# RapidAI/RapidDoc

Measured on AMD Instinct MI355X. Metric: pages/sec (layout+OCR det/rec), higher is better.
Workload: dtype f32

## Files before the change

### include/rapiddoc_mi355.h

```cpp
#ifndef RAPIDDOC_MI355_H
#define RAPIDDOC_MI355_H

#include <stddef.h>
#include <stdint.h>

#ifdef __cplusplus
extern "C" {
#endif

typedef struct rd_handle rd_handle;

#define RD_REC_UNFUSED_CTC 1
#define RD_REC_WANT_SOFTMAX 2
#define RD_REC_WANT_LOGITS 4
#define RD_REC_WANT_NECK 64

const char* rd_version(void);
rd_handle* rd_create(int device_id, const char* model_kind);
const char* rd_create_error(void);
void rd_destroy(rd_handle* h);
const char* rd_last_error(rd_handle* h);

int rd_load_weights(rd_handle* h, const void* safetensors_image, size_t nbytes);

int rd_query_workspace(rd_handle* h, int B, int H, int W, int flags, size_t* ws_bytes);

int rd_det_forward(rd_handle* h, const float* x_nchw_dev, int B, int H, int W, float* prob_b1hw_dev, void* ws_dev,
                   size_t ws_bytes, void* stream);
#define RD_DET_WANT_NECK 1
int rd_det_forward_ex(rd_handle* h, const float* x_nchw_dev, int B, int H, int W, float* prob_b1hw_dev, int flags, float* aux_dev,
                      void* ws_dev, size_t ws_bytes, void* stream);

int rd_rec_forward(rd_handle* h, const float* x_nchw_dev, int B, int W, int32_t* idx_bt_dev, float* prob_bt_dev,
                   float* full_btc_dev, int flags, void* ws_dev, size_t ws_bytes, void* stream);
int rd_rec_num_classes(rd_handle* h);
#define RD_REC_STAGE_BACKBONE 8
#define RD_REC_STAGE_TAIL 16
int rd_rec_token_dim(rd_handle* h);
int rd_rec_backbone_forward(rd_handle* h, const float* x_nchw_dev, int B, int W, float* tokens_btd_dev, void* ws_dev, size_t ws_bytes,
                            void* stream);
int rd_rec_tail_forward(rd_handle* h, const float* tokens_dev, int n_tokens, int n_lines, int max_tokens, const int32_t* seg_dev,
                        const int32_t* tokinfo_dev, int32_t* idx_dev, float* prob_dev, void* ws_dev, size_t ws_bytes, void* stream);
#define RD_REC_LINE_WIDTHS 32
int rd_rec_backbone_forward_lines(rd_handle* h, const float* x_nchw_dev, int B, int W, const int32_t* line_tab_dev, float* tokens_dev,
                                  void* ws_dev, size_t ws_bytes, void* stream);
int rd_rec_seq_len(int W);

int rd_backbone_forward(rd_handle* h, const float* x_nchw_dev, int B, int H, int W, float* const feats_dev[4],
                        void* ws_dev, size_t ws_bytes, void* stream);

int rd_formula_encoder_forward(rd_handle* h, const float* x_nchw_dev, int B, int C, int H, int W, float* enc_dev,
                               void* ws_dev, size_t ws_bytes, void* stream);

int rd_formula_decode(rd_handle* h, const float* enc_dev, int B, int S, int max_new_tokens, int64_t* ids_dev, int32_t* n_cols,
                      void* stream);
#define RD_FORMULA_STREAM_MAX_SLOTS 32
#define RD_FORMULA_STREAM_MAX_TOKENS 65536
typedef struct rd_formula_stream_stats {
    int32_t steps;
    int32_t live_slot_steps;
    int32_t slots;
    int32_t admitted;
} rd_formula_stream_stats;
int rd_formula_decode_stream(rd_handle* h, const float* enc_dev, int N, int S, int max_new_tokens, int slots, int64_t* ids_dev,
                             int32_t* lens_dev, rd_formula_stream_stats* stats, void* stream);
int rd_formula_max_new_tokens(rd_handle* h);

int rd_preproc_resize_norm(int device_id, const uint8_t* hwc_u8_dev, int H, int W, int OH, int OW, const float mean[3],
                           const float std[3], float scale, int interp, int swap_rb, float* out_chw_dev, void* stream);

int rd_preproc_resize_norm_batch(int device_id, const uint8_t* pages_u8_dev, int P, int H, int W, int OH, int OW, const float mean[3],
                                 const float std[3], float scale, int interp, int swap_rb, float* out_nchw_dev, void* stream);

#define RD_RESIZE_AA_MAX_SIDE 16384
int rd_preproc_resize_aa_norm(int device_id, const uint8_t* hwc_u8_dev, int H, int W, int OH, int OW, const float mean[3],
                              const float std[3], int swap_rb, float* out_chw_dev, uint8_t* out_u8_hwc_dev, void* stream);

#define RD_RESAMPLE_BILINEAR 2
#define RD_RESAMPLE_BICUBIC 3
#define RD_FORMULA_SIDE 384
typedef struct rd_formula_crop {
    const uint8_t* base;
    int64_t pitch;
    int32_t w, h;
} rd_formula_crop;
typedef struct rd_formula_plan {
    int32_t served;
    int32_t resize_w, resize_h;
    int32_t thumb;
    int32_t final_w, final_h;
    int32_t fx, fy;
    int32_t reduced_w, reduced_h;
    float box_w, box_h;
    int32_t pad_x, pad_y;
} rd_formula_plan;
int rd_formula_margin_boxes(int device_id, const rd_formula_crop* descs_dev, int n, int32_t* boxes_dev, void* stream);
int rd_formula_preproc_plan(int w, int h, rd_formula_plan* plan);
int rd_formula_preproc_batch(int device_id, const rd_formula_crop* descs_host, const int32_t* boxes_host, int n, float* out_dev,
                             uint8_t* out_u8_dev, void* stream);

typedef struct rd_crop_desc {
    int32_t page;
    int32_t out_w;
    float crop_w, crop_h;
    float m[9];
    int32_t rot90;
    int32_t pad_;
} rd_crop_desc;
int rd_crop_resize_norm_batch(int device_id, const uint8_t* pages_u8_dev, int P, int H, int W,
                              const rd_crop_desc* descs_dev, int n, int out_h, int out_w_padded, const float mean[3],
                              const float std[3], float scale, int swap_rb, float* out_nchw_dev, void* stream);

typedef struct rd_line_crop_desc {
    int32_t page;
    int32_t out_w;
    int32_t crop_w, crop_h;
    int32_t rot90;
    int32_t scratch_off;
    double m[9];
} rd_line_crop_desc;
int rd_line_crops_batch(int device_id, const uint8_t* pages_u8_dev, int P, int H, int W, const rd_line_crop_desc* descs_dev,
                        int n, int64_t max_crop_pixels, uint8_t* scratch_u8_dev, int out_h, int out_w_padded, int swap_rb,
                        float* out_nchw_dev, void* stream);

int rd_line_warp_batch(int device_id, const uint8_t* pages_u8_dev, int P, int H, int W, const rd_line_crop_desc* descs_dev, int n,
                       int64_t max_crop_pixels, uint8_t* scratch_u8_dev, void* stream);
int rd_line_resize_norm_batch(int device_id, const rd_line_crop_desc* descs_dev, int n, const uint8_t* scratch_u8_dev, int out_h,
                              int out_w_padded, int swap_rb, float* out_nchw_dev, void* stream);

#define RD_CLS_WANT_AUX 1
int rd_cls_forward(rd_handle* h, const float* x_nchw_dev, int B, int H, int W, float* prob_b2_dev, int flags, float* aux_dev, void* ws_dev,
                   size_t ws_bytes, void* stream);
int rd_table_encoder_forward(rd_handle* h, const float* x_nchw_dev, int B, int H, int W, float* memory_bt768_dev, void* ws_dev, size_t ws_bytes,
                             void* stream);
typedef struct {
    int32_t prefix_id, eos_id, pad_id, bbox_close_id, bbox_first_id, bbox_last_id;
} rd_table_decode_cfg;
int rd_table_decode(rd_handle* h, const float* memory_dev, int B, int S, int max_new_tokens, const rd_table_decode_cfg* cfg, int64_t* ids_dev,
                    int32_t* n_tokens, void* stream);
#define RD_TABLE_STREAM_MAX_SLOTS 8
#define RD_TABLE_STREAM_MAX_TOKENS 65536
typedef struct rd_table_stream_stats {
    int32_t steps;
    int32_t live_slot_steps;
    int32_t slots;
    int32_t admitted;
} rd_table_stream_stats;
int rd_table_decode_stream(rd_handle* h, const float* memory_dev, int N, int S, int max_new_tokens, int slots, const rd_table_decode_cfg* cfg,
                           int64_t* ids_dev, int32_t* lens_dev, rd_table_stream_stats* stats, void* stream);
int rd_line_flip180_batch(int device_id, const rd_line_crop_desc* descs_dev, int n, const float* cls_prob_n2_dev, float thresh,
                          uint8_t* scratch_u8_dev, int32_t* flipped_out_dev, void* stream);

int rd_ctc_collapse(int device_id, const int32_t* idx_bt_dev, const float* prob_bt_dev, int B, int T, const uint8_t* char_table_dev,
                    int max_len, int n_classes, uint8_t* out_dev, int row_bytes, void* stream);
int rd_ctc_collapse_lines(int device_id, const int32_t* idx_dev, const float* prob_dev, int n_lines, const int32_t* seg_dev, int max_tokens,
                          const uint8_t* char_table_dev, int max_len, int n_classes, uint8_t* out_dev, int row_bytes, uint16_t* kept_cols_dev,
                          float* kept_conf_dev, void* stream);
int rd_ctc_rows_text(const uint8_t* rows_host, int n, int row_bytes, uint8_t* text_out, int64_t text_cap, int64_t* byte_off_out,
                     int32_t* n_chars_out, double* conf_out, double* conf3_out);

typedef struct rd_text_box {
    float pts[8];
    float score;
} rd_text_box;
int rd_db_postprocess(const float* prob_host, int B, int H, int W, const int32_t* src_hw, float thresh, float box_thresh,
                      float unclip_ratio, int use_dilation, int max_candidates, rd_text_box* out, int max_out,
                      int32_t* n_out, int n_threads);

size_t rd_db_boxes_workspace(int B, int H, int W, int max_runs, int max_candidates);
int rd_db_boxes_device(int device_id, const float* prob_dev, int B, int H, int W, const int32_t* src_hw_dev, float thresh, float box_thresh,
                       float unclip_ratio, int use_dilation, int max_candidates, int max_runs, void* ws_dev, size_t ws_bytes,
                       rd_text_box* out_dev, int max_out, int32_t* n_out_dev, void* stream);

int rd_text_boxes_order_merge(const rd_text_box* boxes, const int32_t* counts, int B, int max_in, float* quads_out, int32_t* n_out);

typedef struct rd_layout_post_cfg {
    int32_t n_classes;
    int32_t image_index, formula_index;
    int32_t thresh_is_dict;
    const float* thresh;
    int32_t layout_nms;
    int32_t merge_kind;
    const int8_t* merge_per_class;
    int32_t unclip_kind;
    const float* unclip;
    const uint8_t* unclip_present;
} rd_layout_post_cfg;
int rd_layout_postprocess(const float* boxes, int n, int ncol, int img_w, int img_h, const rd_layout_post_cfg* cfg,
                          float* out, int32_t* out_order, int32_t* n_out);
int rd_layout_postprocess_select(const float* boxes, int n, int ncol, int img_w, int img_h, const rd_layout_post_cfg* cfg,
                                 float* sel_boxes, int32_t* sel_src, int32_t* n_sel);

int rd_msdeform_attn(int device_id, const float* value, const int32_t* shapes, const int32_t* level_start, const float* loc, const float* attn,
                     float* out, int B, int S, int H, int D, int Q, int L, int P, void* stream);
int rd_topk_rows(int device_id, const float* scores, int rows, int n, int k, float* out_vals, int32_t* out_idx, void* stream);
size_t rd_encoder_layer_workspace(int M, int Dm, int F);
int rd_encoder_layer(int device_id, const float* x, const float* pos, int B, int T, int Dm, int heads, int F, int act, const float* in_w,
                     const float* in_b, const float* out_w, const float* out_b, const float* ln1_g, const float* ln1_b, const float* w1,
                     const float* b1, const float* w2, const float* b2, const float* ln2_g, const float* ln2_b, float eps, float* out, void* ws,
                     size_t ws_bytes, void* stream);

int rd_find_external_contours(const uint8_t* mask, int h, int w, int32_t* pts_out, int max_pts, int32_t* counts_out, int max_contours,
                              int32_t* n_contours, int32_t* n_pts);
double rd_contour_area(const int32_t* pts, int n);
double rd_arc_length(const int32_t* pts, int n, int closed);
int rd_approx_poly_dp(const int32_t* pts, int n, double epsilon, int closed, int32_t* out, int32_t* n_out);
int rd_min_area_rect_points(const float* pts, int n, float* out8);
double rd_polygon_area(const double* a, int na);
double rd_polygon_intersection_area(const double* a, int na, const double* b, int nb);
int rd_fill_poly(uint8_t* img, int h, int w, const int32_t* pts, int n, int value);

int rd_find_external_contours_none(const uint8_t* mask, int h, int w, int32_t* pts_out, int max_pts, int32_t* counts_out, int max_contours,
                                   int32_t* n_contours, int32_t* n_pts);

#define RD_CHECKBOX_MAX_SIDE 16384
#define RD_CHECKBOX_MAX_PAGES 1024
#define RD_CHECKBOX_ROI_ROWS 70
#define RD_CHECKBOX_WS_PARTS 13
#define RD_CHECKBOX_RUNS_OVERFLOW 1
#define RD_CHECKBOX_CANDS_OVERFLOW 2
typedef struct rd_checkbox_page {
    int32_t n_runs;
    int32_t flags;
    int32_t n_comp;
    int32_t n_cand;
    int32_t first_key;
    int32_t cand_off;
    int32_t reserved[2];
} rd_checkbox_page;
typedef struct rd_checkbox_cand {
    int32_t key;
    int32_t tick;
    int16_t x, y, w, h;
    int16_t rx, ry, rw, rh;
    uint64_t roi[RD_CHECKBOX_ROI_ROWS];
} rd_checkbox_cand;
typedef struct rd_checkbox_box { int32_t x, y, w, h, ticked; } rd_checkbox_box;
size_t rd_checkbox_workspace(int P, int H, int W, int max_runs, int max_cand, size_t* offsets);
int rd_checkbox_detect_device(int device_id, const uint8_t* pages_dev, int P, int H, int W, int bgr, int max_runs, int max_cand, void* ws_dev,
                              size_t ws_bytes, rd_checkbox_page* hdr_dev, rd_checkbox_cand* cands_dev, void* stream);
int rd_checkbox_finish(const rd_checkbox_cand* cands, int n, int H, int W, rd_checkbox_box* out, int max_out, int32_t* n_out);

#define RD_REGION_MAX_POLY 64
typedef struct rd_region_desc {
    const uint8_t* page;
    int64_t pitch;
    int32_t page_w, page_h;
    int32_t x0, y0, x1, y1;
    int32_t paste_x, paste_y;
    int32_t poly_off, poly_n;
    int32_t box_off, box_n;
} rd_region_desc;
size_t rd_region_canvases_workspace(int n, int gh, int gw);
int rd_region_canvases(int device_id, const rd_region_desc* descs_dev, int n, const int32_t* pts_dev, const int32_t* boxes_dev,
                       int gh, int gw, uint8_t* canv_dev, uint8_t* det_canv_dev , void* ws_dev, size_t ws_bytes, void* stream);

int rd_stage_pack(const uint8_t* const* srcs, const int64_t* pitches, const int32_t* hs, const int32_t* ws, const int64_t* offsets, int n,
                  uint8_t* dst, int64_t dst_bytes, int n_threads);

#define RD_STAGE_SWAP_RB 1u
typedef struct rd_stage_desc {
    const uint8_t* src;
    int64_t pitch;
    uint8_t* canvas;
    int32_t w, h;
    int32_t gh, gw;
    uint32_t flags;
    uint32_t reserved;
} rd_stage_desc;
int rd_stage_canvases(int device_id, const rd_stage_desc* descs_host, const rd_stage_desc* descs_dev, int n, void* stream);

double rd_rec_chunk_cost(int n_lines, int wpad, int n_cu);
int rd_rec_plan_chunks(const int32_t* wpad_sorted, int n, int n_min, int n_max, int n_step, int n_cu, int32_t* sizes_out, int max_out,
                       int32_t* n_out);
int rd_rec_plan_lines(const double* ratios, const int64_t* order, int n, int rec_batch_num, int img_h, int img_w, int launch_multiple,
                      int n_min, int n_max, int n_step, int n_cu, int64_t* line_w_out, double* line_ratio_out, int32_t* sizes_out,
                      int32_t* launch_w_out, int max_out, int32_t* n_out);

int rd_set_precision(rd_handle* h, const char* mode);
int rd_range_status(rd_handle* h, void* stream);

int rd_plan_stats(rd_handle* h, uint64_t* plans_built, uint64_t* graph_captures, uint64_t* graph_replays);

int rd_set_profiling(rd_handle* h, int on);
const char* rd_profile_json(rd_handle* h);

#ifdef __cplusplus
}
#endif
#endif
```

### rapiddoc_amd/_lib.py

```python
from __future__ import annotations

import ctypes as C
from pathlib import Path

_PKG = Path(__file__).resolve().parent
LIB_PATH = _PKG / "librapiddoc_mi355.so"
_lib = None

SYMBOLS = {
    "rd_version": (C.c_char_p, []),
    "rd_create": (C.c_void_p, [C.c_int, C.c_char_p]),
    "rd_create_error": (C.c_char_p, []),
    "rd_destroy": (None, [C.c_void_p]),
    "rd_last_error": (C.c_char_p, [C.c_void_p]),
    "rd_load_weights": (C.c_int, [C.c_void_p, C.c_void_p, C.c_size_t]),
    "rd_query_workspace": (C.c_int, [C.c_void_p, C.c_int, C.c_int, C.c_int, C.c_int, C.POINTER(C.c_size_t)]),
    "rd_det_forward": (C.c_int, [C.c_void_p, C.c_void_p, C.c_int, C.c_int, C.c_int, C.c_void_p, C.c_void_p, C.c_size_t, C.c_void_p]),
    "rd_det_forward_ex": (C.c_int, [C.c_void_p, C.c_void_p, C.c_int, C.c_int, C.c_int, C.c_void_p, C.c_int, C.c_void_p, C.c_void_p, C.c_size_t, C.c_void_p]),
    "rd_rec_forward": (C.c_int, [C.c_void_p, C.c_void_p, C.c_int, C.c_int, C.c_void_p, C.c_void_p, C.c_void_p, C.c_int, C.c_void_p, C.c_size_t, C.c_void_p]),
    "rd_rec_num_classes": (C.c_int, [C.c_void_p]),
    "rd_rec_token_dim": (C.c_int, [C.c_void_p]),
    "rd_rec_backbone_forward": (C.c_int, [C.c_void_p, C.c_void_p, C.c_int, C.c_int, C.c_void_p, C.c_void_p, C.c_size_t, C.c_void_p]),
    "rd_rec_backbone_forward_lines": (C.c_int, [C.c_void_p, C.c_void_p, C.c_int, C.c_int, C.c_void_p, C.c_void_p, C.c_void_p, C.c_size_t, C.c_void_p]),
    "rd_rec_tail_forward": (C.c_int, [C.c_void_p, C.c_void_p, C.c_int, C.c_int, C.c_int, C.c_void_p, C.c_void_p, C.c_void_p, C.c_void_p,
                                      C.c_void_p, C.c_size_t, C.c_void_p]),
    "rd_rec_seq_len": (C.c_int, [C.c_int]),
    "rd_backbone_forward": (C.c_int, [C.c_void_p, C.c_void_p, C.c_int, C.c_int, C.c_int, C.POINTER(C.c_void_p), C.c_void_p, C.c_size_t, C.c_void_p]),
    "rd_formula_encoder_forward": (C.c_int, [C.c_void_p, C.c_void_p, C.c_int, C.c_int, C.c_int, C.c_int, C.c_void_p, C.c_void_p, C.c_size_t, C.c_void_p]),
    "rd_formula_decode": (C.c_int, [C.c_void_p, C.c_void_p, C.c_int, C.c_int, C.c_int, C.c_void_p, C.POINTER(C.c_int32), C.c_void_p]),
    "rd_formula_decode_stream": (C.c_int, [C.c_void_p, C.c_void_p, C.c_int, C.c_int, C.c_int, C.c_int, C.c_void_p, C.c_void_p, C.c_void_p, C.c_void_p]),
    "rd_formula_max_new_tokens": (C.c_int, [C.c_void_p]),
    "rd_preproc_resize_norm": (C.c_int, [C.c_int, C.c_void_p, C.c_int, C.c_int, C.c_int, C.c_int, C.POINTER(C.c_float), C.POINTER(C.c_float), C.c_float, C.c_int, C.c_int, C.c_void_p, C.c_void_p]),
    "rd_preproc_resize_norm_batch": (C.c_int, [C.c_int, C.c_void_p, C.c_int, C.c_int, C.c_int, C.c_int, C.c_int, C.POINTER(C.c_float), C.POINTER(C.c_float), C.c_float, C.c_int, C.c_int, C.c_void_p, C.c_void_p]),
    "rd_preproc_resize_aa_norm": (C.c_int, [C.c_int, C.c_void_p, C.c_int, C.c_int, C.c_int, C.c_int, C.POINTER(C.c_float), C.POINTER(C.c_float), C.c_int, C.c_void_p, C.c_void_p, C.c_void_p]),
    "rd_formula_margin_boxes": (C.c_int, [C.c_int, C.c_void_p, C.c_int, C.c_void_p, C.c_void_p]),
    "rd_formula_preproc_plan": (C.c_int, [C.c_int, C.c_int, C.c_void_p]),
    "rd_formula_preproc_batch": (C.c_int, [C.c_int, C.c_void_p, C.c_void_p, C.c_int, C.c_void_p, C.c_void_p, C.c_void_p]),
    "rd_crop_resize_norm_batch": (C.c_int, [C.c_int, C.c_void_p, C.c_int, C.c_int, C.c_int, C.c_void_p, C.c_int, C.c_int, C.c_int, C.POINTER(C.c_float), C.POINTER(C.c_float), C.c_float, C.c_int, C.c_void_p, C.c_void_p]),
    "rd_line_crops_batch": (C.c_int, [C.c_int, C.c_void_p, C.c_int, C.c_int, C.c_int, C.c_void_p, C.c_int, C.c_int64, C.c_void_p, C.c_int, C.c_int, C.c_int, C.c_void_p, C.c_void_p]),
    "rd_line_warp_batch": (C.c_int, [C.c_int, C.c_void_p, C.c_int, C.c_int, C.c_int, C.c_void_p, C.c_int, C.c_int64, C.c_void_p, C.c_void_p]),
    "rd_line_resize_norm_batch": (C.c_int, [C.c_int, C.c_void_p, C.c_int, C.c_void_p, C.c_int, C.c_int, C.c_int, C.c_void_p, C.c_void_p]),
    "rd_cls_forward": (C.c_int, [C.c_void_p, C.c_void_p, C.c_int, C.c_int, C.c_int, C.c_void_p, C.c_int, C.c_void_p, C.c_void_p, C.c_size_t, C.c_void_p]),
    "rd_table_encoder_forward": (C.c_int, [C.c_void_p, C.c_void_p, C.c_int, C.c_int, C.c_int, C.c_void_p, C.c_void_p, C.c_size_t, C.c_void_p]),
    "rd_table_decode": (C.c_int, [C.c_void_p, C.c_void_p, C.c_int, C.c_int, C.c_int, C.c_void_p, C.c_void_p, C.c_void_p, C.c_void_p]),
    "rd_table_decode_stream": (C.c_int, [C.c_void_p, C.c_void_p, C.c_int, C.c_int, C.c_int, C.c_int, C.c_void_p, C.c_void_p, C.c_void_p, C.c_void_p, C.c_void_p]),
    "rd_line_flip180_batch": (C.c_int, [C.c_int, C.c_void_p, C.c_int, C.c_void_p, C.c_float, C.c_void_p, C.c_void_p, C.c_void_p]),
    "rd_ctc_collapse": (C.c_int, [C.c_int, C.c_void_p, C.c_void_p, C.c_int, C.c_int, C.c_void_p, C.c_int, C.c_int, C.c_void_p, C.c_int, C.c_void_p]),
    "rd_ctc_collapse_lines": (C.c_int, [C.c_int, C.c_void_p, C.c_void_p, C.c_int, C.c_void_p, C.c_int, C.c_void_p, C.c_int, C.c_int, C.c_void_p, C.c_int, C.c_void_p, C.c_void_p,
                                        C.c_void_p]),
    "rd_db_postprocess": (C.c_int, [C.c_void_p, C.c_int, C.c_int, C.c_int, C.c_void_p, C.c_float, C.c_float, C.c_float, C.c_int, C.c_int, C.c_void_p, C.c_int, C.c_void_p, C.c_int]),
    "rd_db_boxes_workspace": (C.c_size_t, [C.c_int, C.c_int, C.c_int, C.c_int, C.c_int]),
    "rd_db_boxes_device": (C.c_int, [C.c_int, C.c_void_p, C.c_int, C.c_int, C.c_int, C.c_void_p, C.c_float, C.c_float, C.c_float, C.c_int, C.c_int,
                                     C.c_int, C.c_void_p, C.c_size_t, C.c_void_p, C.c_int, C.c_void_p, C.c_void_p]),
    "rd_rec_chunk_cost": (C.c_double, [C.c_int, C.c_int, C.c_int]),
    "rd_rec_plan_chunks": (C.c_int, [C.c_void_p, C.c_int, C.c_int, C.c_int, C.c_int, C.c_int, C.c_void_p, C.c_int, C.c_void_p]),
    "rd_rec_plan_lines": (C.c_int, [C.c_void_p, C.c_void_p] + [C.c_int] * 9 + [C.c_void_p] * 4 + [C.c_int, C.c_void_p]),
    "rd_text_boxes_order_merge": (C.c_int, [C.c_void_p, C.c_void_p, C.c_int, C.c_int, C.c_void_p, C.c_void_p]),
    "rd_ctc_rows_text": (C.c_int, [C.c_void_p, C.c_int, C.c_int, C.c_void_p, C.c_int64, C.c_void_p, C.c_void_p, C.c_void_p, C.c_void_p]),
    "rd_layout_postprocess": (C.c_int, [C.c_void_p, C.c_int, C.c_int, C.c_int, C.c_int, C.c_void_p, C.c_void_p, C.c_void_p, C.c_void_p]),
    "rd_layout_postprocess_select": (C.c_int, [C.c_void_p, C.c_int, C.c_int, C.c_int, C.c_int, C.c_void_p, C.c_void_p, C.c_void_p, C.c_void_p]),
    "rd_find_external_contours": (C.c_int, [C.c_void_p, C.c_int, C.c_int, C.c_void_p, C.c_int, C.c_void_p, C.c_int, C.c_void_p, C.c_void_p]),
    "rd_find_external_contours_none": (C.c_int, [C.c_void_p, C.c_int, C.c_int, C.c_void_p, C.c_int, C.c_void_p, C.c_int, C.c_void_p, C.c_void_p]),
    "rd_checkbox_workspace": (C.c_size_t, [C.c_int, C.c_int, C.c_int, C.c_int, C.c_int, C.c_void_p]),
    "rd_checkbox_detect_device": (C.c_int, [C.c_int, C.c_void_p, C.c_int, C.c_int, C.c_int, C.c_int, C.c_int, C.c_int, C.c_void_p, C.c_size_t, C.c_void_p,
                                            C.c_void_p, C.c_void_p]),
    "rd_checkbox_finish": (C.c_int, [C.c_void_p, C.c_int, C.c_int, C.c_int, C.c_void_p, C.c_int, C.c_void_p]),
    "rd_region_canvases_workspace": (C.c_size_t, [C.c_int, C.c_int, C.c_int]),
    "rd_region_canvases": (C.c_int, [C.c_int, C.c_void_p, C.c_int, C.c_void_p, C.c_void_p, C.c_int, C.c_int, C.c_void_p, C.c_void_p, C.c_void_p, C.c_size_t,
                                     C.c_void_p]),
    "rd_stage_pack": (C.c_int, [C.c_void_p, C.c_void_p, C.c_void_p, C.c_void_p, C.c_void_p, C.c_int, C.c_void_p, C.c_int64, C.c_int]),
    "rd_stage_canvases": (C.c_int, [C.c_int, C.c_void_p, C.c_void_p, C.c_int, C.c_void_p]),
    "rd_contour_area": (C.c_double, [C.c_void_p, C.c_int]),
    "rd_arc_length": (C.c_double, [C.c_void_p, C.c_int, C.c_int]),
    "rd_approx_poly_dp": (C.c_int, [C.c_void_p, C.c_int, C.c_double, C.c_int, C.c_void_p, C.c_void_p]),
    "rd_min_area_rect_points": (C.c_int, [C.c_void_p, C.c_int, C.c_void_p]),
    "rd_polygon_area": (C.c_double, [C.c_void_p, C.c_int]),
    "rd_polygon_intersection_area": (C.c_double, [C.c_void_p, C.c_int, C.c_void_p, C.c_int]),
    "rd_fill_poly": (C.c_int, [C.c_void_p, C.c_int, C.c_int, C.c_void_p, C.c_int, C.c_int]),
    "rd_msdeform_attn": (C.c_int, [C.c_int] + [C.c_void_p] * 6 + [C.c_int] * 7 + [C.c_void_p]),
    "rd_topk_rows": (C.c_int, [C.c_int, C.c_void_p, C.c_int, C.c_int, C.c_int, C.c_void_p, C.c_void_p, C.c_void_p]),
    "rd_encoder_layer_workspace": (C.c_size_t, [C.c_int, C.c_int, C.c_int]),
    "rd_encoder_layer": (C.c_int, [C.c_int, C.c_void_p, C.c_void_p] + [C.c_int] * 6 + [C.c_void_p] * 12 + [C.c_float, C.c_void_p, C.c_void_p, C.c_size_t, C.c_void_p]),
    "rd_set_precision": (C.c_int, [C.c_void_p, C.c_char_p]),
    "rd_range_status": (C.c_int, [C.c_void_p, C.c_void_p]),
    "rd_plan_stats": (C.c_int, [C.c_void_p, C.POINTER(C.c_uint64), C.POINTER(C.c_uint64), C.POINTER(C.c_uint64)]),
    "rd_set_profiling": (C.c_int, [C.c_void_p, C.c_int]),
    "rd_profile_json": (C.c_char_p, [C.c_void_p]),
}

_I, _P, _F = C.c_int, C.c_void_p, C.c_float
DEBUG_SYMBOLS = {
    "rd_debug_det_forward_stages": (_I, [_P, _P, _I, _I, _I, _P, _P, _P]),
    "rd_debug_cls_forward_stages": (_I, [_P, _P, _I, _I, _I, _P, _P, _P, _P]),
    "rd_debug_table_decode": (_I, [_P, _P, _I, _I, _I, _P] + [_P] * 7),
    "rd_debug_table_decode_stream": (_I, [_P, _P, _I, _I, _I, _I, _P, _P, _P, _P, _P, _P, _P, _P, _I]),
    "rd_debug_table_encoder_taps": (_I, [_P, _P, _I, _I, _I, _P, _P, _P]),
    "rd_debug_formula_decode": (_I, [_P, _P, _I, _I, _I, _P, C.POINTER(C.c_int32), _P, _P, _P]),
    "rd_debug_formula_decode_stream": (_I, [_P, _P, _I, _I, _I, _I, _P, _P, _P, _P, _P, _P, _P, _I]),
    "rd_debug_resize_aa_coeffs": (_I, [_I, _I, _P, _P, C.c_int64]),
    "rd_debug_resample_coeffs": (_I, [_I, _I, C.c_double, C.c_double, _I, _P, _P, C.c_int64]),
    "rd_debug_region_keep_mask": (_I, [_I, _I, _P, _I, _P]),
    "rd_debug_time_mixer": (_F, [_I] * 4 + [_P] * 6),
    "rd_debug_time_gemm": (_F, [_I] * 5 + [_P] * 6),
    "rd_debug_gemm_h1": (_F, [_I] * 5 + [_P, _I, _P, _P, _P, _I, _P, _I, _P]),
    "rd_debug_seqconv": (_F, [_I] * 8 + [_P, _I, _P, _I, _P, _P, _P, _P, _I, _P]),
    "rd_debug_det_local": (_F, [_I] * 5 + [_P] * 5 + [_F, _P, C.POINTER(C.c_int)]),
    "rd_debug_conv_route": (_I, [_I] * 17 + [_P, _I]),
    "rd_debug_conv_ex": (_F, [_I] * 22 + [_P] * 10 + [C.c_char_p, _P, _I, _P]),
    "rd_debug_conv": (_F, [_I] * 14 + [_P] * 8),
    "rd_debug_stem34": (_F, [_I] * 11 + [_P] * 7),
    "rd_debug_dwconv_ex": (_F, [_I] * 17 + [_P] * 10 + [_I]),
    "rd_debug_dwconv": (_F, [_I] * 8 + [_P] * 8),
    "rd_debug_dw_route": (_I, [_I] * 9 + [_P, _I, _P]),
    "rd_debug_weight_split": (_I, [_P, _I, _I, _P, _P]),
    "rd_debug_lcv3_dw": (_F, [_I] * 9 + [_P] * 8),
    "rd_debug_dw5_strip": (_F, [_I] * 11 + [_P] * 7),
    "rd_debug_mv1e_pool": (_I, [_I] * 4 + [_P] * 3),
    "rd_debug_derived_tensor": (C.c_long, [C.c_char_p, C.c_char_p, C.c_size_t, C.c_char_p, _P, C.c_long]),
    "rd_debug_mbv3_dw": (_F, [_I] * 12 + [_P] * 4),
    "rd_debug_mbv3_block": (_F, [_I] * 14 + [_P] * 8),
    "rd_debug_mbv3_block_ok": (_I, [_I] * 12),
    "rd_debug_mbv3s_dw": (_F, [_I] * 13 + [_P] * 4),
    "rd_debug_mbv3s_block": (_F, [_I] * 15 + [_P] * 12),
    "rd_debug_lcv3_dw_det": (_F, [_I] * 10 + [_P] * 5),
    "rd_debug_lcv3_block": (_F, [_I] * 9 + [_P] * 9),
    "rd_debug_time_ctc": (_F, [_I] * 4 + [_P] * 7 + [_I, _P]),
    "rd_debug_time_checkbox_mask": (_F, [_I] * 4 + [_P, _P]),
    "rd_debug_attention": (_I, [_I] * 4 + [_F, _P, _P, _P, _I, _P]),
    "rd_debug_vit_attention": (_I, [_I] * 4 + [_F, _P, _P]),
    "rd_debug_attention_limits": (_I, [_I, _P, _P]),
    "rd_debug_layernorm": (_I, [_I, _I, _P, _I, _P, _I, _P, _P, _F]),
    "rd_debug_se_chain": (_I, [_I] * 7 + [_F] + [_I] * 3 + [_P] * 9),
    "rd_debug_maxpool2x2s1": (_I, [_I] * 6 + [_P] * 2),
    "rd_debug_avgpool3x2": (_I, [_I] * 6 + [_P] * 3),
    "rd_debug_mask_cols": (_I, [_I] * 5 + [_P, _P, _I]),
    "rd_debug_upsample": (_I, [_I] * 8 + [_P] * 2),
    "rd_debug_add": (_I, [_I] * 5 + [_P] * 3),
    "rd_debug_det_head_tail": (_I, [_I] * 4 + [_P] * 6),
    "rd_debug_ctc_head": (_I, [_I] * 3 + [_P, _I] + [_P] * 6 + [_I, _P, _P]),
    "rd_debug_dec_gemv": (_I, [_I] * 4 + [_P] * 7),
    "rd_debug_dec_attention": (_I, [_I] * 4 + [_P, _P, _I, C.c_longlong] + [_P] * 5 + [_P, _I, _P, _P, _I, _P, _I]),
    "rd_debug_dec_select": (_I, [_I, _P, _I, _I, _I, _P, _I, _P, _I, _I] + [_P] * 6),
}


class NativeLibraryError(RuntimeError):
    pass


def load():
    global _lib
    if _lib is not None:
        return _lib
    if not LIB_PATH.exists():
        raise NativeLibraryError(
            f"{LIB_PATH} is missing - build it with `python -m rapiddoc_amd.build` (hipcc, gfx950). "
            "rapiddoc_amd has no CPU fallback.")
    import torch
    lib = C.CDLL(str(LIB_PATH))
    for name, (res, args) in {**SYMBOLS, **DEBUG_SYMBOLS}.items():
        fn = getattr(lib, name)
        fn.restype = res
        fn.argtypes = args
    _lib = lib
    return lib
```

### rapiddoc_amd/build.py

```python
from __future__ import annotations

import os
import shutil
import subprocess
import sys
from concurrent.futures import ThreadPoolExecutor
from pathlib import Path

PKG = Path(__file__).resolve().parent
CSRC = PKG / "csrc"
OUT = PKG / "librapiddoc_mi355.so"
SOURCES = ["kernels_conv.hip", "kernels_conv_h3.hip", "kernels_conv_direct_h3.hip", "kernels_conv3x3_h1.hip", "kernels_conv9x9_h1.hip", "kernels_stem34.hip", "kernels_rtdetr.hip", "kernels_conv_stream_h3.hip", "kernels_gemm_h3_dma.hip", "kernels_gemm_h1.hip", "kernels_misc.hip", "kernels_dw_lds.hip", "kernels_stem_fused.hip", "kernels_image.hip", "kernels_resize_aa.hip", "kernels_dbpost.hip", "kernels_checkbox.hip", "kernels_region.hip", "kernels_stage.hip", "kernels_attention_h3.hip", "kernels_seqconv.hip", "kernels_det_local.hip", "kernels_lcv3.hip", "kernels_lcv3_det.hip", "kernels_mv1e.hip", "kernels_mbv3.hip", "kernels_mbv3s.hip", "kernels_vit_attn.hip", "kernels_lcv3_block.hip", "kernels_ctc.hip", "kernels_mixer.hip", "kernels_mixer_h3.hip", "kernels_mixer_ws.hip", "kernels_mixer_res.hip", "formula_decoder.hip", "table_decoder.hip", "engine.cpp", "builder.cpp", "builder_mobile.cpp", "models.cpp", "api.cpp", "api_debug.cpp", "db_postprocess.cpp", "layout_postprocess.cpp", "polygon_ops.cpp", "checkbox_host.cpp", "rec_chunks.cpp", "host_stages.cpp", "stage_pack.cpp"]
FLAGS = ["--offload-arch=gfx950", "-O3", "-std=c++17", "-fPIC", "-Wall", "-Wno-unused-function", "-x", "hip"]
FILE_FLAGS = {"kernels_mixer_ws.hip": ["-fno-slp-vectorize", "-DRD_GELU_SCALAR"], "kernels_gemm_h1.hip": ["-fno-slp-vectorize"],
              "kernels_stem_fused.hip": ["-fno-slp-vectorize"]}


def extra_flags_for(src: str) -> list:
    return list(FILE_FLAGS.get(Path(src).name, []))


def _hipcc() -> str:
    for cand in (os.environ.get("HIPCC"), shutil.which("hipcc"), "/opt/rocm/bin/hipcc"):
        if cand and Path(cand).exists():
            return cand
    raise RuntimeError("hipcc not found (ROCm 7.x required)")


def needs_build() -> bool:
    if not OUT.exists():
        return True
    t = OUT.stat().st_mtime
    deps = list(CSRC.glob("*")) + [PKG.parent / "include" / "rapiddoc_mi355.h", Path(__file__)]
    return any(d.stat().st_mtime > t for d in deps)


def build(force: bool = False, verbose: bool = True, extra_flags: tuple = (), out: Path = None) -> Path:
    variant = out is not None
    if not variant and not force and not needs_build():
        return OUT
    hipcc = _hipcc()
    objdir = PKG / "build" / (Path(out).stem if variant else "")
    objdir.mkdir(parents=True, exist_ok=True)
    OUT_ = Path(out) if variant else OUT

    def compile_one(src: str) -> Path:
        obj = objdir / (src + ".o")
        cmd = [hipcc, *FLAGS, *extra_flags_for(src), *extra_flags, "-c", str(CSRC / src), "-o", str(obj)]
        r = subprocess.run(cmd, capture_output=True, text=True)
        if r.returncode != 0:
            raise RuntimeError(f"hipcc failed for {src}:\n{r.stdout}\n{r.stderr}")
        if verbose and r.stderr.strip():
            print(r.stderr, file=sys.stderr)
        return obj

    with ThreadPoolExecutor(max_workers=min(8, len(SOURCES))) as ex:
        objs = list(ex.map(compile_one, SOURCES))
    tmp = OUT_.with_name(OUT_.name + f".tmp{os.getpid()}")
    cmd = [hipcc, "--offload-arch=gfx950", "-shared", "-fPIC", *map(str, objs), "-o", str(tmp)]
    r = subprocess.run(cmd, capture_output=True, text=True)
    if r.returncode != 0:
        tmp.unlink(missing_ok=True)
        raise RuntimeError(f"link failed:\n{r.stdout}\n{r.stderr}")
    os.replace(tmp, OUT_)
    if verbose:
        print(f"built {OUT_} ({OUT_.stat().st_size/1e6:.1f} MB)")
    return OUT_


if __name__ == "__main__":
    build(force="--force" in sys.argv)
```

### rapiddoc_amd/pipeline.py

```python
from __future__ import annotations

import os
import time
import ctypes as C
from concurrent.futures import ThreadPoolExecutor
from dataclasses import dataclass, field
from typing import Dict, List, Optional, Sequence, Tuple

import numpy as np
import torch

from . import _lib, ocr_host
from .engine import RdEngine, preproc_resize_norm, preproc_resize_norm_batch
from .rec_plan import (CLS_IMG_H, CLS_IMG_W, LINE_DTYPE, RecPlan, plan_rec,
                       quad_to_crop_matrix, quads_to_crop_matrices)

LAYOUT_SIZE = 800
DET_LIMIT = 960


class CropDesc(C.Structure):
    _fields_ = [("page", C.c_int32), ("out_w", C.c_int32), ("crop_w", C.c_float), ("crop_h", C.c_float),
                ("m", C.c_float * 9), ("rot90", C.c_int32), ("pad_", C.c_int32)]


def cls_flip_rule(prob: np.ndarray, thresh: float) -> np.ndarray:
    p = np.asarray(prob, dtype=np.float32).reshape(-1, 2)
    return (p[:, 1] > p[:, 0]) & (p[:, 1] >= np.float32(thresh))


def flip180(crop: np.ndarray) -> np.ndarray:
    return np.ascontiguousarray(np.asarray(crop)[::-1, ::-1])


CROP_DTYPE = np.dtype([("page", "<i4"), ("out_w", "<i4"), ("crop_w", "<f4"), ("crop_h", "<f4"), ("m", "<f4", (9,)),
                       ("rot90", "<i4"), ("pad_", "<i4")])
assert CROP_DTYPE.itemsize == C.sizeof(CropDesc)


def boxes_to_quads(boxes_xyxy: np.ndarray) -> np.ndarray:
    b = np.asarray(boxes_xyxy, dtype=np.float32).reshape(-1, 4)
    return np.stack([b[:, [0, 1]], b[:, [2, 1]], b[:, [2, 3]], b[:, [0, 3]]], axis=1)


@dataclass
class PageResult:
    lines: List[Tuple[np.ndarray, str, float]] = field(default_factory=list)
    layout_feats: Optional[List[torch.Tensor]] = None
    cls: Optional[List[Tuple[bool, int, float]]] = None


@dataclass(slots=True)
class _RecLaunch:
    x: Optional[torch.Tensor] = None
    event: Optional[torch.cuda.Event] = None
    done: Optional[torch.cuda.Event] = None
    idx: Optional[torch.Tensor] = None
    prob: Optional[torch.Tensor] = None
    rows: Optional[torch.Tensor] = None
    cols: Optional[Tuple[torch.Tensor, torch.Tensor]] = None
    cls_prob: Optional[torch.Tensor] = None
    cls_flip: Optional[torch.Tensor] = None


class PagePipeline:
    def __init__(self, states: Dict[str, object], device: int = 0, characters: Optional[Sequence[str]] = None,
                 rec_batch_num: Optional[int] = None, rec_width_multiple: int = 32, keep_feats: bool = False, n_rec_streams: int = 4,
                 rec_mode: Optional[str] = None, rec_chunking: Optional[str] = None, use_cls: bool = False, cls_thresh: float = 0.9):
        self.use_cls, self.cls_thresh = bool(use_cls), float(cls_thresh)
        if self.use_cls and "ppocr_cls_mobile" not in states:
            raise ValueError("use_cls=True needs the text-line classifier's weights: states['ppocr_cls_mobile'] (ch_ptocr_mobile_v2.0_cls_mobile)")
        if rec_mode is None:
            rec_mode = "strict" if rec_batch_num is None and rec_chunking is None else "throughput"
        if rec_mode not in ("strict", "throughput"):
            raise ValueError("rec_mode must be 'strict' or 'throughput'")
        if rec_chunking is None:
            rec_chunking = "adaptive" if rec_batch_num is None else "fixed"
        if rec_batch_num is None:
            rec_batch_num = 64
        if rec_chunking not in ("fixed", "adaptive"):
            raise ValueError("rec_chunking must be 'fixed' or 'adaptive'")
        self.rec_mode = rec_mode
        self.rec_chunking = rec_chunking
        if rec_mode == "strict":
            rec_batch_num, rec_width_multiple = 6, 1
        self.device = device
        self.tdev = torch.device("cuda", device)
        self.n_cu = int(torch.cuda.get_device_properties(self.tdev).multi_processor_count)
        det_kinds = [k for k in ("ppocrv6_det", "ppocrv5_det_server", "ppocrv5_det_mobile", "ppocrv3_det_mobile") if k in states]
        if len(det_kinds) != 1:
            raise ValueError("states must carry exactly one detector: 'ppocrv6_det' or 'ppocrv5_det_server' or 'ppocrv5_det_mobile' or 'ppocrv3_det_mobile'")
        self.det_kind = det_kinds[0]
        self.det = RdEngine(self.det_kind, device, guard="deferred", reuse_outputs=True).load_weights(states[self.det_kind])
        rec_kinds = [k for k in ("ppocrv6_rec", "ppocrv5_rec_server", "ppocrv5_rec_mobile", "ppocr_rec_mv1e") if k in states]
        if len(rec_kinds) != 1:
            raise ValueError("states must carry exactly one recogniser: 'ppocrv6_rec' or 'ppocrv5_rec_server' or 'ppocrv5_rec_mobile' or 'ppocr_rec_mv1e'")
        self.rec_kind = rec_kinds[0]
        self.rec_lines_in_launch = self.rec_kind in ("ppocrv6_rec", "ppocrv5_rec_mobile", "ppocr_rec_mv1e")
        self.rec_engines = [RdEngine(self.rec_kind, device, guard="deferred").load_weights(states[self.rec_kind]) for _ in range(max(1, n_rec_streams))]
        self.rec = self.rec_engines[0]
        self.rec_streams = [torch.cuda.Stream(device=self.tdev) for _ in self.rec_engines]
        self.rec_tail = RdEngine(self.rec_kind, device, guard="deferred").load_weights(states[self.rec_kind])
        self.cls_engines = ([RdEngine("ppocr_cls_mobile", device, guard="deferred").load_weights(states["ppocr_cls_mobile"]) for _ in self.rec_engines]
                            if self.use_cls else [])
        self.last_cls = None
        self.tail_stream = torch.cuda.Stream(device=self.tdev)
        self.layout_stream = torch.cuda.Stream(device=self.tdev)
        self.front_stream = torch.cuda.Stream(device=self.tdev)
        self._prefetched: Optional[dict] = None
        self._after_rec_enqueue = None
        self.prefetch_gate = float(os.environ.get("RD_PREFETCH_GATE", "1.0"))
        self.layout = RdEngine("pphgnetv2_b4", device, guard="deferred", reuse_outputs=True).load_weights(states["pphgnetv2_b4"]) if "pphgnetv2_b4" in states else None
        self._bufs: Dict[tuple, torch.Tensor] = {}
        ncls = self.rec.num_classes
        self.characters = list(characters) if characters is not None else ["blank"] + [chr(0x4E00 + i) for i in range(ncls - 2)] + [" "]
        assert len(self.characters) == ncls, (len(self.characters), ncls)
        self.rec_batch_num = rec_batch_num
        self.rec_width_multiple = rec_width_multiple
        self.keep_feats = keep_feats
        tab, self._ctc_max_len = ocr_host.char_table(self.characters)
        self._ctc_table = torch.from_numpy(tab).to(self.tdev)
        self.device_ctc = True
        self.device_db = True
        self.host_native = ocr_host.host_native_default()
        self.db_ws: dict = {}
        self.rec_two_stage = os.environ.get("RD_REC_TWO_STAGE", "1") != "0"
        self.rec_width_sync = None
        self._sync_this_call = True
        self._width_sync_cache = None
        self._width_sync_epoch, self._in_run_batch = 0, False
        self.keep_rec_inputs = False
        self.last_rec_batches: List[Tuple[np.ndarray, torch.Tensor, torch.Tensor, torch.Tensor]] = []
        self._lib = _lib.load()
        self.stats: Dict[str, float] = {}

    def _buf(self, role, numel: int, dtype=torch.float32) -> torch.Tensor:
        key = (role, dtype)
        t = self._bufs.get(key)
        if t is None or t.numel() < numel:
            t = self._bufs[key] = torch.empty(int(numel * 1.25) + 64, dtype=dtype, device=self.tdev)
        return t[:numel]

    def layout_preprocess(self, pages: torch.Tensor) -> torch.Tensor:
        P = pages.shape[0]
        out = self._buf("layout_x", P * 3 * LAYOUT_SIZE * LAYOUT_SIZE).view(P, 3, LAYOUT_SIZE, LAYOUT_SIZE)
        return preproc_resize_norm_batch(pages, (LAYOUT_SIZE, LAYOUT_SIZE), interp=2, out=out)

    def layout_forward(self, pages: torch.Tensor) -> List[torch.Tensor]:
        return self.layout.backbone_forward(self.layout_preprocess(pages))

    def det_preprocess(self, pages: torch.Tensor) -> Tuple[torch.Tensor, Tuple[int, int]]:
        P, H, W, _ = pages.shape
        bh, bw = -(-(H + 100) // 64) * 64, -(-(W + 100) // 64) * 64
        dh, dw = ocr_host.det_resize_shape(bh, bw, DET_LIMIT, "max")
        out = self._buf("det_x", P * 3 * dh * dw).view(P, 3, dh, dw)
        x = preproc_resize_norm_batch(pages, (dh, dw), mean=ocr_host.DET_MEAN, std=ocr_host.DET_STD, interp=1, swap_rb=True, out=out)
        return x, (dh, dw)

    def det_forward(self, pages: torch.Tensor) -> Tuple[torch.Tensor, Tuple[int, int]]:
        x, det_hw = self.det_preprocess(pages)
        return self.det.det_forward(x), det_hw

    def rec_forward_lines(self, pages: torch.Tensor, quads_per_page: Sequence[np.ndarray]):
        return self.rec_forward_sources([(pages, quads_per_page)])[0]

    def rec_forward_sources(self, sources: Sequence[Tuple[torch.Tensor, Sequence[np.ndarray]]],
                            image_keys: Optional[Sequence[Sequence[int]]] = None, want_words: bool = False,
                            pooled: bool = True):
        self._sync_this_call = bool(pooled)
        if not self._in_run_batch:
            self._width_sync_epoch += 1
        out = self._rec_forward_sources_once(sources, image_keys, want_words)
        for _ in range(3):
            if not any([e.check_range_and_fallback() for e in self.rec_engines + [self.rec_tail] + self.cls_engines]):
                break
            self.stats["range_fallbacks"] = self.stats.get("range_fallbacks", 0) + 1
            out = self._rec_forward_sources_once(sources, image_keys, want_words)
        return out

    def _synced_widths(self, sync, keys: np.ndarray, ratios: np.ndarray):
        sig = (self._width_sync_epoch, keys.tobytes(), ratios.tobytes())
        if self._width_sync_cache is not None and self._width_sync_cache[0] == sig:
            return self._width_sync_cache[1]
        res = sync(keys, ratios)
        self._width_sync_cache = (sig, res)
        return res

    def _collapse_home(self, name: str, n: int, T: int, call, *extra: torch.Tensor) -> List[torch.Tensor]:
        row_bytes = (16 + T * self._ctc_max_len + 15) // 16 * 16
        rows = torch.empty((n, row_bytes), dtype=torch.uint8, device=self.tdev)
        if call(rows.data_ptr(), row_bytes) != 0:
            raise RuntimeError(f"{name} failed")
        home = []
        for t in (rows,) + extra:
            h = torch.empty(t.shape, dtype=t.dtype, pin_memory=True)
            h.copy_(t, non_blocking=True)
            home.append(h)
        return home

    def _collapse_rows(self, idx: torch.Tensor, prob: torch.Tensor, nb: int, st, record: bool = True):
        rows = done = None
        with torch.cuda.stream(st):
            if self.device_ctc:
                T = idx.shape[1]
                rows, = self._collapse_home("rd_ctc_collapse", nb, T, lambda out, row_bytes: self._lib.rd_ctc_collapse(
                    self.device, idx.data_ptr(), prob.data_ptr(), nb, T, self._ctc_table.data_ptr(), self._ctc_max_len, len(self.characters),
                    out, row_bytes, st.cuda_stream))
            if record:
                done = torch.cuda.Event()
                done.record(st)
        return rows, done

    def _collapse_lines(self, idx_all: torch.Tensor, prob_all: torch.Tensor, tables: torch.Tensor, n_lines: int, max_tokens: int, st,
                        want_cols: bool = False):
        with torch.cuda.stream(st):
            cols = torch.empty((n_lines, max_tokens), dtype=torch.int16, device=self.tdev) if want_cols else None
            confs = torch.empty((n_lines, max_tokens), dtype=torch.float32, device=self.tdev) if want_cols else None
            rows, *cols_h = self._collapse_home("rd_ctc_collapse_lines", n_lines, max_tokens, lambda out, row_bytes: self._lib.rd_ctc_collapse_lines(
                self.device, idx_all.data_ptr(), prob_all.data_ptr(), n_lines, tables.data_ptr(), max_tokens, self._ctc_table.data_ptr(),
                self._ctc_max_len, len(self.characters), out, row_bytes, cols.data_ptr() if want_cols else None,
                confs.data_ptr() if want_cols else None, st.cuda_stream), *((cols, confs) if want_cols else ()))
            done = torch.cuda.Event()
            done.record(st)
        return rows, done, tuple(cols_h) if want_cols else None

    def _rec_forward_sources_once(self, sources, image_keys=None, want_words=False):
        t0 = time.perf_counter()
        if self.use_cls and want_words:
            raise ValueError("use_cls together with want_words: rapidocr defines no word-box mapping for lines turned by 180 degrees")
        self.last_cls = None
        for imgs, _quads in sources:
            assert imgs.is_cuda and imgs.dtype == torch.uint8 and imgs.dim() == 4 and imgs.is_contiguous()
        strict = self.rec_mode == "strict"
        sync = None
        if self.rec_width_sync is not None and strict and self.rec_two_stage and self._sync_this_call:
            sync = lambda keys, ratios: self._synced_widths(self.rec_width_sync, keys, ratios)
        plan = plan_rec([(imgs.shape[0], quads) for imgs, quads in sources], image_keys, strict=strict, two_stage=self.rec_two_stage,
                        lines_in_launch=self.rec_lines_in_launch, chunking=self.rec_chunking, rec_batch_num=self.rec_batch_num,
                        rec_width_multiple=self.rec_width_multiple, n_cu=self.n_cu, n_streams=len(self.rec_engines), use_cls=self.use_cls,
                        host_native=self.host_native, want_words=want_words, width_sync=sync)
        scatter = lambda per_line: self._scatter_texts(per_line, plan.src_of, plan.page_of, plan.n_img, plan.perm)
        cls_of: List[tuple] = [(False, 0, 0.0)] * plan.n_all
        if plan.n == 0:
            if self.use_cls and plan.n_all:
                self.last_cls = scatter(cls_of)
            return scatter([("", 0.0, None) if want_words else ("", 0.0)] * plan.n_all)
        if getattr(self, "_crop_scratch", None) is None or self._crop_scratch.numel() < plan.scratch_bytes:
            self._crop_scratch = torch.empty(int(plan.scratch_bytes * 1.25) + 1024, dtype=torch.uint8, device=sources[0][0].device)
        self.stats["t_descs_ms"] = (time.perf_counter() - t0) * 1e3
        main = torch.cuda.current_stream()
        launches = self._enqueue_rec(plan, sources, want_words)
        self.stats["t_rec_enqueue_ms"] = (time.perf_counter() - t0) * 1e3 - self.stats["t_descs_ms"]
        hook, self._after_rec_enqueue = self._after_rec_enqueue, None
        if hook is not None:
            t_h = time.perf_counter()
            S, nb = len(self.rec_engines), len(launches)
            m = max(1, min(nb, int(np.ceil(self.prefetch_gate * nb))))
            hook([l.event for l in launches[max(0, m - S): m]])
            self.stats["t_front_next_ms"] = (time.perf_counter() - t_h) * 1e3
        texts = self._decode_rec(plan, launches, want_words)
        for st in self.rec_streams + [self.tail_stream]:
            main.wait_stream(st)
        self.stats["rec_lines"] = plan.n
        self.stats["rec_batches"] = len(launches)
        self.last_pool_order = plan.perm
        if self.use_cls:
            ph = np.concatenate([l.cls_prob.numpy() for l in launches])
            fh = np.concatenate([l.cls_flip.numpy() for l in launches])
            for j, i in enumerate(plan.line_ids.tolist()):
                label = int(ph[j, 1] > ph[j, 0])
                cls_of[i] = (bool(fh[j]), label, float(ph[j, label]))
            self.last_cls = scatter(cls_of)
            self.last_cls_prob = (plan.line_ids, ph)
        return scatter(texts)

    def _enqueue_rec(self, plan: RecPlan, sources, want_words: bool) -> List[_RecLaunch]:
        dev, S, lib = sources[0][0].device, len(self.rec_engines), self._lib
        keep_inputs = self.keep_rec_inputs
        upload = lambda descs: torch.from_numpy(descs.view(np.uint8)).to(dev, non_blocking=True)
        descs_dev = upload(plan.descs)
        cls = None
        if self.use_cls:
            cls = (upload(plan.descs_cls), self._buf("cls_prob", 2 * plan.n).view(plan.n, 2), self._buf("cls_flip", plan.n, torch.int32),
                   torch.empty((plan.n, 2), dtype=torch.float32, pin_memory=True), torch.empty((plan.n,), dtype=torch.int32, pin_memory=True))
        descs_warp_dev = upload(plan.descs_warp) if plan.descs_warp is not None else descs_dev
        if keep_inputs:
            self.last_rec_descs = (plan.descs.copy(), np.asarray(plan.batch_base, dtype=np.int64), np.asarray(plan.starts, dtype=np.int64))
            self.last_cls_inputs = []
        main = torch.cuda.current_stream()
        ready = torch.cuda.Event()
        ready.record(main)
        tokens = linetab = tables = None
        if plan.two_stage:
            base = plan.group_base
            tokens = self._buf("rec_tokens", int(base[-1]) * self.rec.rec_token_dim).view(int(base[-1]), self.rec.rec_token_dim)
            for gi, lens in enumerate(plan.group_lens):
                tokens[int(base[gi]) + int(lens.sum()): int(base[gi + 1])].zero_()
            tables = [self.rec_tail.rec_tail_tables(lp, dev, out=self._buf(("tail_tab", gi), 2 * len(lp) + int(lp.sum()), torch.int32))
                      for gi, (lp, _t) in enumerate(plan.group_pad)]
            if plan.linetab is not None:
                tab_h = torch.from_numpy(plan.linetab).pin_memory()
                linetab = self._buf("rec_linetab", 4 * plan.n, torch.int32).view(plan.n, 4)
                linetab.copy_(tab_h, non_blocking=True)
                self._keep_linetab = tab_h
            ready.record(main)
            self.tail_stream.wait_event(ready)
        launches: List[_RecLaunch] = []
        for bi, (chunk, wpad) in enumerate(plan.batches):
            nb, pos = len(chunk), int(plan.starts[bi])
            k = bi % S
            st = self.rec_streams[k]
            if bi < S:
                st.wait_event(ready)
            with torch.cuda.stream(st):
                x = self._buf(("rec_x", k), nb * 3 * ocr_host.REC_IMG_H * wpad).view(nb, 3, ocr_host.REC_IMG_H, wpad)
                scratch = self._crop_scratch.data_ptr() + int(plan.batch_base[bi])
                for si, first, cnt, max_px in plan.warp_jobs[bi]:
                    imgs = sources[si][0]
                    rc = lib.rd_line_warp_batch(self.device, imgs.data_ptr(), imgs.shape[0], imgs.shape[1], imgs.shape[2],
                                                descs_warp_dev.data_ptr() + first * LINE_DTYPE.itemsize, cnt, max_px, scratch, st.cuda_stream)
                    if rc != 0:
                        raise RuntimeError("rd_line_warp_batch failed")
                launch = _RecLaunch()
                if cls is not None:
                    self._enqueue_cls(launch, cls, descs_dev, k, pos, nb, scratch, plan.line_ids[pos: pos + nb])
                rc = lib.rd_line_resize_norm_batch(self.device, descs_dev.data_ptr() + pos * LINE_DTYPE.itemsize, nb, scratch,
                                                   ocr_host.REC_IMG_H, wpad, 1, x.data_ptr(), st.cuda_stream)
                if rc != 0:
                    raise RuntimeError("rd_line_resize_norm_batch failed")
                if plan.lines_in_launch:
                    self.rec_engines[k].rec_backbone_forward_lines(x, linetab[pos: pos + nb], tokens)
                elif plan.two_stage:
                    self.rec_engines[k].rec_backbone_forward(x, tokens[plan.tok_lo[bi]: plan.tok_lo[bi] + nb * int(plan.seq_line[pos])])
                else:
                    launch.idx, launch.prob, _ = self.rec_engines[k].rec_forward(x)
                    launch.rows, launch.done = self._collapse_rows(launch.idx, launch.prob, nb, st)
                launch.event = launch.done
                if plan.two_stage:
                    launch.event = torch.cuda.Event()
                    launch.event.record(st)
                launch.x = x.clone() if keep_inputs else x
            launches.append(launch)
            if plan.two_stage and ((bi + 1) % S == 0 or bi + 1 == len(plan.batches)):
                self._enqueue_tail(plan, launches, bi // S, tokens, tables[bi // S], want_words)
        return launches

    def _enqueue_cls(self, launch: _RecLaunch, cls, descs_dev, k: int, pos: int, nb: int, scratch: int, line_ids: np.ndarray) -> None:
        descs_cls_dev, cls_prob, cls_flip, cls_prob_h, cls_flip_h = cls
        stream = torch.cuda.current_stream().cuda_stream
        sl = slice(pos, pos + nb)
        xc = self._buf(("cls_x", k), nb * 3 * CLS_IMG_H * CLS_IMG_W).view(nb, 3, CLS_IMG_H, CLS_IMG_W)
        rc = self._lib.rd_line_resize_norm_batch(self.device, descs_cls_dev.data_ptr() + pos * LINE_DTYPE.itemsize, nb, scratch,
                                                 CLS_IMG_H, CLS_IMG_W, 1, xc.data_ptr(), stream)
        if rc != 0:
            raise RuntimeError("rd_line_resize_norm_batch (classifier) failed")
        self.cls_engines[k].cls_forward(xc, out=cls_prob[sl])
        if self.keep_rec_inputs:
            self.last_cls_inputs.append((line_ids, xc.clone()))
        rc = self._lib.rd_line_flip180_batch(self.device, descs_dev.data_ptr() + pos * LINE_DTYPE.itemsize, nb, cls_prob[sl].data_ptr(),
                                             self.cls_thresh, scratch, cls_flip[sl].data_ptr(), stream)
        if rc != 0:
            raise RuntimeError("rd_line_flip180_batch failed")
        launch.cls_prob, launch.cls_flip = cls_prob_h[sl], cls_flip_h[sl]
        launch.cls_prob.copy_(cls_prob[sl], non_blocking=True)
        launch.cls_flip.copy_(cls_flip[sl], non_blocking=True)

    def _enqueue_tail(self, plan: RecPlan, launches: List[_RecLaunch], gi: int, tokens: torch.Tensor, tables: torch.Tensor, want_words: bool) -> None:
        grp = [launches[bi] for bi in plan.groups[gi]]
        t_lo, t_hi = int(plan.group_base[gi]), int(plan.group_base[gi + 1])
        lens_pad, max_tokens = plan.group_pad[gi]
        for launch in grp:
            self.tail_stream.wait_event(launch.event)
        with torch.cuda.stream(self.tail_stream):
            n_tok = t_hi - t_lo
            idx_all, prob_all = self.rec_tail.rec_tail_forward(
                tokens[t_lo:t_hi], lens_pad, tables, max_tokens=max_tokens,
                out=(self._buf(("tail_idx", gi), n_tok, torch.int32), self._buf(("tail_prob", gi), n_tok)))
        done = None
        if plan.lines_mode:
            last = grp[-1]
            last.rows, done, last.cols = self._collapse_lines(idx_all, prob_all, tables, len(plan.group_lens[gi]), max_tokens, self.tail_stream,
                                                              want_words)
            if self.keep_rec_inputs:
                with torch.cuda.stream(self.tail_stream):
                    last.idx, last.prob = idx_all.clone(), prob_all.clone()
        else:
            for bi, launch in zip(plan.groups[gi], grp):
                nb, t = len(plan.batches[bi][0]), int(plan.seq_line[int(plan.starts[bi])])
                lo = plan.tok_lo[bi] - t_lo
                launch.idx, launch.prob = idx_all[lo: lo + nb * t].view(nb, t), prob_all[lo: lo + nb * t].view(nb, t)
                launch.rows, ev = self._collapse_rows(launch.idx, launch.prob, nb, self.tail_stream, record=launch is grp[-1])
                done = ev or done
        for launch in grp:
            launch.done = done

    def _texts_from_rows(self, rows_np: np.ndarray, line_ids: np.ndarray, texts: list) -> None:
        if self.host_native:
            txt, _conf, conf3 = ocr_host.parse_ctc_rows_native(rows_np)
            for i, t, s in zip(line_ids.tolist(), txt, conf3):
                texts[i] = (t, s)
        else:
            for i, (t, s) in zip(line_ids.tolist(), ocr_host.parse_ctc_rows(rows_np)):
                texts[i] = (t, ocr_host.format_score(s))

    def _words_from_rows(self, plan: RecPlan, lo: int, rows_np: np.ndarray, cols, texts: list) -> None:
        n_kept = rows_np[:, 8:12].copy().view("<i4")[:, 0]
        cols_np, confs_np = cols[0].numpy(), cols[1].numpy()
        for j, (t, sc) in enumerate(ocr_host.parse_ctc_rows(rows_np)):
            i, k = int(plan.order_all[lo + j]), int(n_kept[j])
            words = {"cols": cols_np[j, :k].astype(np.int64).tolist(), "confs": confs_np[j, :k].astype(np.float64).tolist(),
                     "n_steps": int(plan.seq_line[lo + j]), "wh_ratio": float(plan.ratios[i]), "max_wh_ratio": float(plan.line_ratio[lo + j]),
                     "crop_hw": (int(plan.eff_h[i]), int(plan.eff_w[i]))}
            texts[int(plan.keep[i])] = (t, sc, words)

    def _decode_groups(self, plan: RecPlan, launches: List[_RecLaunch], want_words: bool, texts: list) -> list:
        ids, starts = plan.line_ids, plan.starts
        t_dec = 0.0
        for gi, grp in enumerate(plan.groups):
            tail = launches[grp[-1]]
            tail.done.synchronize()
            t1 = time.perf_counter()
            lo, hi = int(starts[grp[0]]), int(starts[grp[-1] + 1])
            if want_words:
                self._words_from_rows(plan, lo, tail.rows.numpy(), tail.cols, texts)
            else:
                self._texts_from_rows(tail.rows.numpy(), ids[lo:hi], texts)
            t_dec += time.perf_counter() - t1
            if tail.idx is not None:
                g0 = int(plan.group_base[gi])
                for bi in grp:
                    a, e = int(starts[bi]), int(starts[bi + 1])
                    sl = [(int(plan.first_tok[i]) - g0, int(plan.seq_line[i])) for i in range(a, e)]
                    self.last_rec_batches.append((ids[a:e], launches[bi].x, np.asarray(plan.line_w[a:e]),
                                                  [tail.idx[o: o + t] for o, t in sl], [tail.prob[o: o + t] for o, t in sl]))
        self.stats["t_decode_ms"] = t_dec * 1e3
        return texts

    def _decode_rec(self, plan: RecPlan, launches: List[_RecLaunch], want_words: bool) -> list:
        texts: List[tuple] = [("", 0.0, None) if want_words else ("", 0.0)] * plan.n_all
        ids, starts = plan.line_ids, plan.starts
        t_dec = 0.0
        if self.keep_rec_inputs:
            self.last_rec_crop_sizes = (plan.crop_w.astype(np.int64), plan.crop_h.astype(np.int64), plan.rot90, plan.keep)
        if self.keep_rec_inputs or plan.lines_mode:
            self.last_rec_batches = []
        if plan.lines_mode:
            return self._decode_groups(plan, launches, want_words, texts)
        for bi, launch in enumerate(launches):
            ids_b = ids[int(starts[bi]): int(starts[bi + 1])]
            if self.keep_rec_inputs:
                self.last_rec_batches.append((ids_b, launch.x, launch.idx, launch.prob))
            launch.done.synchronize()
            if launch.rows is not None:
                t1 = time.perf_counter()
                self._texts_from_rows(launch.rows.numpy(), ids_b, texts)
            else:
                idx_h, prob_h = launch.idx.cpu().numpy(), launch.prob.cpu().numpy()
                t1 = time.perf_counter()
                for i, (t, s) in zip(ids_b.tolist(), ocr_host.ctc_decode(idx_h, prob_h, self.characters)):
                    texts[i] = (t, ocr_host.format_score(s))
            t_dec += time.perf_counter() - t1
        self.stats["t_decode_ms"] = t_dec * 1e3
        return texts

    @staticmethod
    def _scatter_texts(texts, src_of, page_of, n_img, perm=None):
        if perm is not None:
            inv = np.argsort(perm, kind="stable")
            texts = [texts[i] for i in inv.tolist()]
            src_of, page_of = src_of[inv], page_of[inv]
        out = [[[] for _ in range(k)] for k in n_img]
        for t, si, pi in zip(texts, src_of.tolist(), page_of.tolist()):
            out[si][pi].append(t)
        return out

    def boxes_from_maps(self, maps_host: np.ndarray, page_hw: Tuple[int, int], box_thresh: float = 0.3,
                        unclip_ratio: float = 1.8) -> List[np.ndarray]:
        P = maps_host.shape[0]
        res = ocr_host.db_postprocess(maps_host, [page_hw] * P, thresh=0.3, box_thresh=box_thresh, unclip_ratio=unclip_ratio,
                                      raw=self.host_native)
        t0 = time.perf_counter()
        if self.host_native:
            out = ocr_host.order_merge_boxes_native(*res)
            self.stats["t_boxes_ms"] = (time.perf_counter() - t0) * 1e3
            return out
        out = []
        for boxes, _scores in res:
            if len(boxes) == 0:
                out.append(np.zeros((0, 4, 2), np.float32))
                continue
            b = ocr_host.sorted_boxes(boxes.astype(np.float32))
            b = ocr_host.merge_det_boxes(b)
            out.append(np.asarray(b, dtype=np.float32).reshape(-1, 4, 2))
        self.stats["t_boxes_ms"] = (time.perf_counter() - t0) * 1e3
        return out

    def boxes_from_maps_device(self, maps_dev: torch.Tensor, page_hw: Tuple[int, int], box_thresh: float = 0.3,
                               unclip_ratio: float = 1.8) -> List[np.ndarray]:
        P = maps_dev.shape[0]
        res = ocr_host.db_postprocess_device(maps_dev, [page_hw] * P, thresh=0.3, box_thresh=box_thresh, unclip_ratio=unclip_ratio,
                                             stats=self.stats, cache=self.db_ws, raw=self.host_native)
        t0 = time.perf_counter()
        if self.host_native:
            out = ocr_host.order_merge_boxes_native(*res)
            self.stats["t_boxes_ms"] = (time.perf_counter() - t0) * 1e3
            return out
        out = []
        for boxes, _scores in res:
            if len(boxes) == 0:
                out.append(np.zeros((0, 4, 2), np.float32))
                continue
            b = ocr_host.merge_det_boxes(ocr_host.sorted_boxes(boxes.astype(np.float32)))
            out.append(np.asarray(b, dtype=np.float32).reshape(-1, 4, 2))
        self.stats["t_boxes_ms"] = (time.perf_counter() - t0) * 1e3
        return out

    def _boxes_via_host_maps(self, src: torch.Tensor, page_hw: Tuple[int, int]) -> List[np.ndarray]:
        if getattr(self, "_maps_host", None) is None or self._maps_host.shape != src.shape:
            self._maps_host = torch.empty(src.shape, dtype=torch.float32, pin_memory=True)
        t0 = time.perf_counter()
        self._maps_host.copy_(src, non_blocking=True)
        torch.cuda.current_stream().synchronize()
        t1 = time.perf_counter()
        quads = self.boxes_from_maps(self._maps_host.numpy(), page_hw)
        self.stats["t_wait_maps_ms"] = (t1 - t0) * 1e3
        self.stats["t_db_post_ms"] = (time.perf_counter() - t1) * 1e3 - self.stats["t_boxes_ms"]
        return quads

    def run_batch(self, pages: torch.Tensor, quads_per_page: Optional[Sequence[np.ndarray]] = None,
                  det_maps_override: Optional[torch.Tensor] = None, prefetch: Optional[torch.Tensor] = None,
                  page_keys: Optional[Sequence[int]] = None) -> List[PageResult]:
        if isinstance(pages, np.ndarray) or not pages.is_cuda:
            src = torch.from_numpy(np.ascontiguousarray(pages)) if isinstance(pages, np.ndarray) else pages.contiguous()
            pages = src.to(self.tdev, non_blocking=src.is_pinned())
        self._page_keys = None if page_keys is None else [int(k) for k in page_keys]
        assert self._page_keys is None or len(self._page_keys) == pages.shape[0]
        if self.rec_width_sync is not None and page_keys is None and getattr(self.rec_width_sync, "world_size", 1) > 1:
            raise ValueError("rec_width_sync over more than one rank needs page_keys: the pages' positions in the GLOBAL page list")
        self._width_sync_epoch += 1
        self._in_run_batch = True
        try:
            return self._run_batch_guarded(pages, quads_per_page, det_maps_override, prefetch)
        finally:
            self._in_run_batch = False

    def _run_batch_guarded(self, pages, quads_per_page, det_maps_override, prefetch):
        results = self._run_batch_once(pages, quads_per_page, det_maps_override, prefetch)
        engines = [self.det] + ([self.layout] if self.layout is not None else [])
        if os.environ.get("RD_DEV_SKIP_RANGE_CHECK") == "1":
            engines = []
        if any([e.check_range_and_fallback() for e in engines]):
            self.stats["range_fallbacks"] = self.stats.get("range_fallbacks", 0) + 1
            self._prefetched = None
            results = self._run_batch_once(pages, quads_per_page, det_maps_override, prefetch)
        return results

    @staticmethod
    def _front_key(pages: torch.Tensor) -> tuple:
        return (pages.data_ptr(), tuple(pages.shape))

    def _front(self, pages: torch.Tensor, n_results: int, gate: Sequence[torch.cuda.Event] = ()) -> dict:
        cur = torch.cuda.current_stream()
        h = {"key": self._front_key(pages), "feats": None, "layout_done": None}
        self.front_stream.wait_stream(cur)
        for ev in gate:
            self.front_stream.wait_event(ev)
        with torch.cuda.stream(self.front_stream):
            h["prob_maps"], h["det_hw"] = self.det_forward(pages)
            h["det_done"] = torch.cuda.Event()
            h["det_done"].record(self.front_stream)
        if self.layout is not None:
            self.layout_stream.wait_event(h["det_done"])
            with torch.cuda.stream(self.layout_stream):
                feats = self.layout_forward(pages)
                if self.keep_feats:
                    h["feats"] = [[f[i].clone() for f in feats] for i in range(n_results)]
                h["layout_done"] = torch.cuda.Event()
                h["layout_done"].record(self.layout_stream)
        return h

    def _run_batch_once(self, pages: torch.Tensor, quads_per_page: Optional[Sequence[np.ndarray]] = None,
                        det_maps_override: Optional[torch.Tensor] = None, prefetch: Optional[torch.Tensor] = None) -> List[PageResult]:
        assert pages.is_cuda and pages.dtype == torch.uint8 and pages.dim() == 4
        P, H, W, _ = pages.shape
        results = [PageResult() for _ in range(P)]
        cur = torch.cuda.current_stream()
        h, self._prefetched = self._prefetched, None
        if h is None or h["key"] != self._front_key(pages):
            h = self._front(pages, P)
            self.stats["front_prefetched"] = 0.0
        else:
            self.stats["front_prefetched"] = 1.0
        cur.wait_event(h["det_done"])
        if self.rec_width_sync is not None and self.det.precision != "fp32" and os.environ.get("RD_DEV_SKIP_RANGE_CHECK") != "1":
            if self.det.check_range_and_fallback():
                self.stats["range_fallbacks"] = self.stats.get("range_fallbacks", 0) + 1
                h = self._front(pages, P)
                self.stats["front_prefetched"] = 0.0
                cur.wait_event(h["det_done"])
        prob_maps, det_hw = h["prob_maps"], h["det_hw"]
        self.last_det = (prob_maps, det_hw)
        if quads_per_page is None:
            src = det_maps_override if det_maps_override is not None else prob_maps
            quads_per_page = self.boxes_from_maps_device(src.contiguous(), (H, W)) if self.device_db else self._boxes_via_host_maps(src, (H, W))
        if prefetch is not None:
            assert prefetch.is_cuda and prefetch.dtype == torch.uint8 and prefetch.dim() == 4

            def front_next(gate):
                self._prefetched = self._front(prefetch, prefetch.shape[0], gate)
            self._after_rec_enqueue = front_next
        try:
            keys = getattr(self, "_page_keys", None)
            texts = self.rec_forward_sources([(pages, quads_per_page)], image_keys=None if keys is None else [keys])[0]
        except BaseException:
            self._after_rec_enqueue = None
            raise
        if self._after_rec_enqueue is not None:
            self._after_rec_enqueue = None
            front_next(())
        if h["layout_done"] is not None:
            cur.wait_event(h["layout_done"])
        for i in range(P):
            qs = np.asarray(quads_per_page[i], dtype=np.float32).reshape(-1, 4, 2)
            results[i].lines = [(qs[j], t, s) for j, (t, s) in enumerate(texts[i])]
            if h["feats"] is not None:
                results[i].layout_feats = h["feats"][i]
            if self.use_cls and self.last_cls is not None:
                results[i].cls = list(self.last_cls[0][i])
        return results


def render_text_maps(boxes_per_page: Sequence[np.ndarray], page_hw: Tuple[int, int], map_hw: Tuple[int, int],
                     device) -> torch.Tensor:
    H, W = page_hw
    h, w = map_hw
    maps = torch.full((len(boxes_per_page), 1, h, w), 0.02, dtype=torch.float32)
    for i, boxes in enumerate(boxes_per_page):
        for x0, y0, x1, y1 in np.asarray(boxes, dtype=np.float64).reshape(-1, 4):
            bw, bh = x1 - x0, y1 - y0
            d = 0.32 * min(bw, bh)
            xa, xb = int(round((x0 + d) * w / W)), int(round((x1 - d) * w / W))
            ya, yb = int(round((y0 + d) * h / H)), int(round((y1 - d) * h / H))
            if xb > xa and yb > ya:
                maps[i, 0, ya:yb, xa:xb] = 0.9
    return maps.to(device)


class PageUploader:

    def __init__(self, device: int = 0, n_buffers: int = 2):
        self.tdev = torch.device("cuda", device)
        self.stream = torch.cuda.Stream(device=self.tdev)
        self.n = max(2, n_buffers)
        self._dev: List[Optional[torch.Tensor]] = [None] * self.n
        self._pin: List[Optional[torch.Tensor]] = [None] * self.n
        self._released: List[Optional[torch.cuda.Event]] = [None] * self.n
        self._consumer: List[Optional[torch.cuda.Stream]] = [None] * self.n
        self._i = 0
        self.bytes_uploaded = 0

    @staticmethod
    def pinned_like(shape) -> torch.Tensor:
        return torch.empty(tuple(shape), dtype=torch.uint8, pin_memory=True)

    def submit(self, pages_host) -> Tuple[torch.Tensor, torch.cuda.Event, int]:
        src = torch.from_numpy(pages_host) if isinstance(pages_host, np.ndarray) else pages_host
        assert not src.is_cuda and src.dtype == torch.uint8 and src.dim() == 4 and src.is_contiguous()
        k = self._i % self.n
        self._i += 1
        if self._dev[k] is None or self._dev[k].numel() < src.numel():
            self._dev[k] = torch.empty(int(src.numel() * 1.1) + 256, dtype=torch.uint8, device=self.tdev)
        dst = self._dev[k][: src.numel()].view(src.shape)
        if self._consumer[k] is not None:
            rel = torch.cuda.Event()
            rel.record(self._consumer[k])
            self._released[k], self._consumer[k] = rel, None
        if self._released[k] is not None:
            self.stream.wait_event(self._released[k])
        if not src.is_pinned():
            if self._pin[k] is None or self._pin[k].numel() < src.numel():
                self._pin[k] = torch.empty(int(src.numel() * 1.1) + 256, dtype=torch.uint8, pin_memory=True)
            self.stream.synchronize()
            stage = self._pin[k][: src.numel()].view(src.shape)
            stage.copy_(src)
            src = stage
        with torch.cuda.stream(self.stream):
            dst.copy_(src, non_blocking=True)
            ev = torch.cuda.Event()
            ev.record(self.stream)
        self.bytes_uploaded += src.numel()
        return dst, ev, k

    def wait(self, ticket: Tuple[torch.Tensor, torch.cuda.Event, int]) -> torch.Tensor:
        dst, ev, k = ticket
        cur = torch.cuda.current_stream()
        cur.wait_event(ev)
        self._consumer[k] = cur
        return dst

    def release(self, ticket) -> None:
        _dst, _ev, k = ticket
        rel = torch.cuda.Event()
        rel.record(torch.cuda.current_stream())
        self._released[k], self._consumer[k] = rel, None


class PagePipelinePool:

    def __init__(self, states: Dict[str, object], device: int = 0, workers: int = 2, **kw):
        self.device = device
        self.pipes = [PagePipeline(states, device, **kw) for _ in range(max(1, workers))]
        self.streams = [torch.cuda.Stream(device=self.pipes[0].tdev) for _ in self.pipes]
        self.pool = ThreadPoolExecutor(max_workers=len(self.pipes))
        self.stats: Dict[str, float] = {}

    @property
    def engines(self) -> List[RdEngine]:
        out = []
        for p in self.pipes:
            out += [p.det, *([p.layout] if p.layout is not None else []), *p.rec_engines, p.rec_tail]
        return out

    def run_batch(self, pages: torch.Tensor, quads_per_page: Optional[Sequence[np.ndarray]] = None,
                  det_maps_override: Optional[torch.Tensor] = None, prefetch: Optional[torch.Tensor] = None,
                  page_keys: Optional[Sequence[int]] = None) -> List[PageResult]:
        assert page_keys is None or len(self.pipes) == 1 or all(p.rec_width_sync is None for p in self.pipes)
        if isinstance(pages, np.ndarray) or not pages.is_cuda:
            src = torch.from_numpy(np.ascontiguousarray(pages)) if isinstance(pages, np.ndarray) else pages.contiguous()
            pages = src.to(self.pipes[0].tdev, non_blocking=src.is_pinned())
        P = pages.shape[0]
        n = min(len(self.pipes), max(1, P))
        bounds = [P * k // n for k in range(n + 1)]
        nb = None
        if prefetch is not None and min(len(self.pipes), max(1, prefetch.shape[0])) == n:
            nb = [prefetch.shape[0] * k // n for k in range(n + 1)]
        ready = torch.cuda.Event()
        ready.record()

        def work(k: int):
            lo, hi = bounds[k], bounds[k + 1]
            torch.cuda.set_device(self.device)
            st = self.streams[k]
            with torch.cuda.stream(st):
                st.wait_event(ready)
                res = self.pipes[k].run_batch(pages[lo:hi], None if quads_per_page is None else quads_per_page[lo:hi],
                                              None if det_maps_override is None else det_maps_override[lo:hi],
                                              None if nb is None else prefetch[nb[k]:nb[k + 1]],
                                              None if page_keys is None else page_keys[lo:hi])
                done = torch.cuda.Event()
                done.record(st)
            return res, done

        outs = list(self.pool.map(work, range(n)))
        results: List[PageResult] = []
        for res, done in outs:
            torch.cuda.current_stream().wait_event(done)
            results += res
        self.stats = {}
        for k, p in enumerate(self.pipes[:n]):
            for key, v in p.stats.items():
                self.stats[key] = self.stats.get(key, 0.0) + v
        return results
```

### rapiddoc_amd/rec_plan.py

```python
from __future__ import annotations

from dataclasses import dataclass
from typing import Callable, List, Optional, Sequence, Tuple

import numpy as np

from . import ocr_host
from .engine import pad_tail_lengths, rec_line_table

CLS_IMG_H, CLS_IMG_W = 48, 192

LINE_DTYPE = np.dtype([("page", "<i4"), ("out_w", "<i4"), ("crop_w", "<i4"), ("crop_h", "<i4"), ("rot90", "<i4"),
                       ("scratch_off", "<i4"), ("m", "<f8", (9,))])
assert LINE_DTYPE.itemsize == 96


def quad_to_crop_matrix(quad: np.ndarray) -> Tuple[np.ndarray, float, float]:
    q = np.asarray(quad, dtype=np.float64).reshape(4, 2)
    cw = max(np.linalg.norm(q[0] - q[1]), np.linalg.norm(q[2] - q[3]))
    ch = max(np.linalg.norm(q[0] - q[3]), np.linalg.norm(q[1] - q[2]))
    cw, ch = float(int(cw)), float(int(ch))
    cw, ch = max(cw, 1.0), max(ch, 1.0)
    src = np.array([[0, 0], [cw, 0], [cw, ch], [0, ch]], dtype=np.float64)
    A, b = [], []
    for (x, y), (u, v) in zip(src, q):
        A.append([x, y, 1, 0, 0, 0, -u * x, -u * y]); b.append(u)
        A.append([0, 0, 0, x, y, 1, -v * x, -v * y]); b.append(v)
    h = np.linalg.solve(np.asarray(A), np.asarray(b))
    return np.append(h, 1.0).astype(np.float32), cw, ch


def quads_to_crop_matrices(quads: np.ndarray) -> Tuple[np.ndarray, np.ndarray, np.ndarray, np.ndarray]:
    q32 = np.asarray(quads, dtype=np.float32).reshape(-1, 4, 2)
    q = q32.astype(np.float64)
    n = len(q)

    def norm32(a, b):
        d = a - b
        return np.sqrt(d[:, 0] * d[:, 0] + d[:, 1] * d[:, 1])
    cw = np.maximum(norm32(q32[:, 0], q32[:, 1]), norm32(q32[:, 2], q32[:, 3])).astype(np.float64)
    ch = np.maximum(norm32(q32[:, 0], q32[:, 3]), norm32(q32[:, 1], q32[:, 2])).astype(np.float64)
    cw, ch = np.floor(cw), np.floor(ch)
    ok = (cw >= 1.0) & (ch >= 1.0) & np.isfinite(cw) & np.isfinite(ch)
    cw, ch = np.where(ok, cw, 1.0), np.where(ok, ch, 1.0)
    z = np.zeros(n)
    src = np.stack([np.stack([z, z], 1), np.stack([cw, z], 1), np.stack([cw, ch], 1), np.stack([z, ch], 1)], axis=1)
    A = np.zeros((n, 8, 8))
    b = np.zeros((n, 8))
    x, y, u, v = src[..., 0], src[..., 1], q[..., 0], q[..., 1]
    A[:, 0::2, 0], A[:, 0::2, 1], A[:, 0::2, 2] = x, y, 1.0
    A[:, 0::2, 6], A[:, 0::2, 7] = -u * x, -u * y
    A[:, 1::2, 3], A[:, 1::2, 4], A[:, 1::2, 5] = x, y, 1.0
    A[:, 1::2, 6], A[:, 1::2, 7] = -v * x, -v * y
    b[:, 0::2], b[:, 1::2] = u, v
    with np.errstate(all="ignore"):
        for i, j, k in ((0, 1, 2), (1, 2, 3), (2, 3, 0), (3, 0, 1)):
            cross = (q[:, j, 0] - q[:, i, 0]) * (q[:, k, 1] - q[:, i, 1]) - (q[:, j, 1] - q[:, i, 1]) * (q[:, k, 0] - q[:, i, 0])
            ok &= np.isfinite(cross) & (np.abs(cross) > 1e-6 * cw * ch)
    A[~ok] = np.eye(8)
    h = np.linalg.solve(A, b[..., None])[..., 0]
    return np.concatenate([h, np.ones((n, 1))], axis=1), cw, ch, ok


@dataclass
class RecPlan:
    n_img: List[int]
    src_of: np.ndarray
    page_of: np.ndarray
    perm: Optional[np.ndarray]
    keep: np.ndarray
    n_all: int
    lines_mode: bool = False
    two_stage: bool = False
    lines_in_launch: bool = False
    crop_w: Optional[np.ndarray] = None
    crop_h: Optional[np.ndarray] = None
    rot90: Optional[np.ndarray] = None
    eff_w: Optional[np.ndarray] = None
    eff_h: Optional[np.ndarray] = None
    ratios: Optional[List[float]] = None
    order_all: Optional[np.ndarray] = None
    line_ids: Optional[np.ndarray] = None
    line_w: Optional[np.ndarray] = None
    line_ratio: Optional[np.ndarray] = None
    batches: Optional[List[Tuple[np.ndarray, int]]] = None
    starts: Optional[np.ndarray] = None
    descs: Optional[np.ndarray] = None
    descs_cls: Optional[np.ndarray] = None
    descs_warp: Optional[np.ndarray] = None
    warp_jobs: Optional[List[List[Tuple[int, int, int, int]]]] = None
    batch_base: Optional[np.ndarray] = None
    seq_line: Optional[np.ndarray] = None
    groups: Optional[List[List[int]]] = None
    group_lens: Optional[List[np.ndarray]] = None
    group_pad: Optional[List[Tuple[np.ndarray, int]]] = None
    group_base: Optional[np.ndarray] = None
    first_tok: Optional[np.ndarray] = None
    tok_lo: Optional[List[int]] = None
    linetab: Optional[np.ndarray] = None

    @property
    def n(self) -> int:
        return len(self.keep)

    @property
    def scratch_bytes(self) -> int:
        return int(self.batch_base[-1])


def _no_lines(sync, **pooling) -> RecPlan:
    if sync is not None:
        sync(np.zeros(0, np.int64), np.zeros(0))
    return RecPlan(**pooling)


def plan_rec(sources: Sequence[Tuple[int, Sequence[np.ndarray]]], image_keys: Optional[Sequence[Sequence[int]]] = None, *,
             strict: bool, two_stage: bool, lines_in_launch: bool, chunking: str, rec_batch_num: int, rec_width_multiple: int,
             n_cu: int, n_streams: int, use_cls: bool = False, host_native: bool = True, want_words: bool = False,
             width_sync: Optional[Callable] = None) -> RecPlan:
    z32 = np.zeros(0, np.int32)
    n_img = [int(k) for k, _q in sources]
    src_of, page_of, quad_list = [], [], []
    for si, (_k, quads_per_img) in enumerate(sources):
        for pi, q in enumerate(quads_per_img):
            q = np.asarray(q, dtype=np.float64).reshape(-1, 4, 2)
            if len(q):
                quad_list.append(q)
                src_of.append(np.full(len(q), si, np.int32))
                page_of.append(np.full(len(q), pi, np.int32))
    if not quad_list:
        return _no_lines(width_sync, n_img=n_img, src_of=z32, page_of=z32, perm=None, keep=np.zeros(0, np.int64), n_all=0)
    quads = np.concatenate(quad_list, axis=0)
    src_of, page_of = np.concatenate(src_of), np.concatenate(page_of)
    perm = None
    if image_keys is not None:
        key = np.array([image_keys[si][pi] for si, pi in zip(src_of.tolist(), page_of.tolist())], dtype=np.int64)
        perm = np.argsort(key, kind="stable")
        quads, src_of, page_of, key = quads[perm], src_of[perm], page_of[perm], key[perm]
    mats, cws_a, chs_a, ok = quads_to_crop_matrices(quads)
    keep = np.nonzero(ok)[0]
    n = len(keep)
    pooling = dict(n_img=n_img, src_of=src_of, page_of=page_of, perm=perm, keep=keep, n_all=len(quads))
    if n == 0:
        return _no_lines(width_sync, **pooling)
    mats, cws_a, chs_a = mats[keep], cws_a[keep], chs_a[keep]
    rots_a = (chs_a / cws_a >= 2.0).astype(np.int32)
    eff_w = np.where(rots_a == 1, chs_a, cws_a)
    eff_h = np.where(rots_a == 1, cws_a, chs_a)
    ratios = (eff_w / eff_h).tolist()
    lines_mode = strict and two_stage
    if want_words and not lines_mode:
        raise RuntimeError("word boxes need the strict two-stage recogniser (rec_mode='strict', RD_REC_TWO_STAGE unset)")
    line_ratio = None
    if lines_mode:
        given = None
        if width_sync is not None:
            line_keys = key[keep] if image_keys is not None else page_of[keep].astype(np.int64)
            given = width_sync(line_keys, np.asarray(ratios, dtype=np.float64))
        batches, line_w, line_ratio = ocr_host.rec_batches_lines(ratios, n_cu=n_cu, with_ratio=True, given=given, native=host_native)
        if not lines_in_launch:
            batches = ocr_host.rec_batches_equal_width(np.concatenate([c for c, _w in batches]), line_w)
    elif not strict and chunking == "adaptive":
        batches = ocr_host.rec_batches_adaptive(ratios, width_multiple=rec_width_multiple, n_cu=n_cu)
    else:
        batches = ocr_host.rec_batches(ratios, rec_batch_num, width_multiple=rec_width_multiple, strict=strict, merge_equal_width=strict)
    order_all = np.concatenate([c for c, _ in batches])
    if not lines_mode:
        line_w = np.concatenate([np.full(len(c), w) for c, w in batches])
    descs = np.zeros(n, dtype=LINE_DTYPE)
    descs["page"] = page_of[keep][order_all]
    descs["out_w"] = np.minimum(line_w, np.ceil(ocr_host.REC_IMG_H * (eff_w / eff_h)[order_all])).astype(np.int32)
    descs["crop_w"] = cws_a[order_all].astype(np.int32)
    descs["crop_h"] = chs_a[order_all].astype(np.int32)
    descs["m"] = mats[order_all]
    descs["rot90"] = rots_a[order_all]
    crop_bytes = (descs["crop_w"].astype(np.int64) * descs["crop_h"] * 3 + 15) // 16 * 16
    nb = len(batches)
    starts = np.cumsum([0] + [len(c) for c, _ in batches])
    offs = np.zeros(n, np.int64)
    batch_scratch = []
    for b in range(nb):
        cb = crop_bytes[starts[b]:starts[b + 1]]
        offs[starts[b]:starts[b + 1]] = np.cumsum(cb) - cb
        batch_scratch.append(int(cb.sum()))
    if max(batch_scratch) >= 2 ** 31:
        raise RuntimeError("a rec batch needs >= 2 GB of crop scratch: lower rec_batch_num")
    descs["scratch_off"] = offs.astype(np.int32)
    plan = RecPlan(**pooling, lines_mode=lines_mode, two_stage=two_stage, lines_in_launch=lines_mode and lines_in_launch,
                   crop_w=cws_a, crop_h=chs_a, rot90=rots_a, eff_w=eff_w, eff_h=eff_h, ratios=ratios,
                   order_all=order_all, line_ids=keep[order_all], line_w=line_w, line_ratio=line_ratio, batches=batches, starts=starts,
                   descs=descs, batch_base=np.cumsum([0] + batch_scratch))
    crop_px = descs["crop_w"].astype(np.int64) * descs["crop_h"]
    plan.warp_jobs = []
    if len(sources) > 1:
        src_sorted = src_of[keep][order_all]
        warp_order = np.concatenate([starts[b] + np.argsort(src_sorted[starts[b]:starts[b + 1]], kind="stable") for b in range(nb)])
        plan.descs_warp = descs[warp_order]
        ws_sorted = src_sorted[warp_order]
        px_sorted = crop_px[warp_order]
        for b in range(nb):
            lo, hi = int(starts[b]), int(starts[b + 1])
            cuts = [lo] + [i for i in range(lo + 1, hi) if ws_sorted[i] != ws_sorted[i - 1]] + [hi]
            plan.warp_jobs.append([(int(ws_sorted[a]), a, e - a, int(px_sorted[a:e].max())) for a, e in zip(cuts[:-1], cuts[1:])])
    else:
        for b in range(nb):
            lo, hi = int(starts[b]), int(starts[b + 1])
            plan.warp_jobs.append([(0, lo, hi - lo, int(crop_px[lo:hi].max()))])
    if use_cls:
        plan.descs_cls = descs.copy()
        plan.descs_cls["out_w"] = np.minimum(CLS_IMG_W, np.ceil(CLS_IMG_H * (eff_w / eff_h)[order_all])).astype(np.int32)
    if two_stage:
        _plan_tokens(plan, n_streams)
    return plan


def _plan_tokens(plan: RecPlan, S: int) -> None:
    starts, nb = plan.starts, len(plan.batches)
    w2_ = (np.asarray(plan.line_w, dtype=np.int64) - 1) // 2 + 1
    seq_line = ((w2_ - 1) // 2 + 1) // 2
    groups = [list(range(g, min(g + S, nb))) for g in range(0, nb, S)]
    plan.group_lens = [seq_line[int(starts[grp[0]]): int(starts[grp[-1] + 1])] for grp in groups]
    plan.group_pad = [pad_tail_lengths(l) for l in plan.group_lens]
    plan.group_base = np.cumsum([0] + [int(lp.sum()) for lp, _t in plan.group_pad])
    first_tok = np.zeros(plan.n, np.int64)
    for gi, grp in enumerate(groups):
        lo, hi = int(starts[grp[0]]), int(starts[grp[-1] + 1])
        first_tok[lo:hi] = int(plan.group_base[gi]) + np.cumsum(seq_line[lo:hi]) - seq_line[lo:hi]
    plan.seq_line, plan.groups, plan.first_tok = seq_line, groups, first_tok
    plan.tok_lo = [int(first_tok[int(starts[bi])]) for bi in range(nb)]
    if plan.lines_in_launch:
        plan.linetab = rec_line_table(plan.line_w, first_tok)
```

Baseline: 374.4.

## Move rec line planning and crop systems into a native C++ planner

Adds a C++ planner that computes crop sizes, perspective systems, keep/rotation/ratios, launch chunks, warp jobs, token groups and packed staging tables in one call. By default it replaces the numpy/Python per-line planning path with a single native call that writes straight into a reusable staging block. The goal is to cut host-side Python overhead between layout/det and rec launches. It adds a second code path that has to match the Python planner's float behaviour exactly, which is why fp contraction is disabled.

```diff
diff --git a/include/rapiddoc_mi355.h b/include/rapiddoc_mi355.h
--- a/include/rapiddoc_mi355.h
+++ b/include/rapiddoc_mi355.h
@@ -277,6 +277,17 @@
                       int n_min, int n_max, int n_step, int n_cu, int64_t* line_w_out, double* line_ratio_out, int32_t* sizes_out,
                       int32_t* launch_w_out, int max_out, int32_t* n_out);
 
+#define RD_REC_PLAN_LINES 0
+#define RD_REC_PLAN_LINES_GIVEN 1
+#define RD_REC_PLAN_ADAPTIVE 2
+#define RD_REC_PLAN_FIXED 3
+int rd_rec_crop_systems(const double* quads, int n, double* cw_out, double* ch_out, uint8_t* ok_out, double* A_out, double* b_out,
+                        int64_t* keep_out, int32_t* rot_out, double* ratio_out, int32_t* n_keep_out);
+int rd_rec_plan(const double* cw, const double* ch, const int32_t* src_of, const int32_t* page_of, const double* mats, int n_all,
+                const int64_t* keep, const int32_t* rot, const double* ratios, const int64_t* order, const int64_t* given_w,
+                const double* given_ratio, int n, const int32_t* cfg, int64_t* line_i64_out, double* line_f64_out, int64_t* launch_out,
+                int64_t* jobs_out, int64_t* group_out, int64_t* meta_out, uint8_t* block, int64_t block_bytes);
+
 int rd_set_precision(rd_handle* h, const char* mode);
 int rd_range_status(rd_handle* h, void* stream);
 
diff --git a/rapiddoc_amd/_lib.py b/rapiddoc_amd/_lib.py
--- a/rapiddoc_amd/_lib.py
+++ b/rapiddoc_amd/_lib.py
@@ -55,6 +55,8 @@
     "rd_rec_chunk_cost": (C.c_double, [C.c_int, C.c_int, C.c_int]),
     "rd_rec_plan_chunks": (C.c_int, [C.c_void_p, C.c_int, C.c_int, C.c_int, C.c_int, C.c_int, C.c_void_p, C.c_int, C.c_void_p]),
     "rd_rec_plan_lines": (C.c_int, [C.c_void_p, C.c_void_p] + [C.c_int] * 9 + [C.c_void_p] * 4 + [C.c_int, C.c_void_p]),
+    "rd_rec_crop_systems": (C.c_int, [C.c_void_p, C.c_int] + [C.c_void_p] * 9),
+    "rd_rec_plan": (C.c_int, [C.c_void_p] * 5 + [C.c_int] + [C.c_void_p] * 6 + [C.c_int] + [C.c_void_p] * 8 + [C.c_int64]),
     "rd_text_boxes_order_merge": (C.c_int, [C.c_void_p, C.c_void_p, C.c_int, C.c_int, C.c_void_p, C.c_void_p]),
     "rd_ctc_rows_text": (C.c_int, [C.c_void_p, C.c_int, C.c_int, C.c_void_p, C.c_int64, C.c_void_p, C.c_void_p, C.c_void_p, C.c_void_p]),
     "rd_layout_postprocess": (C.c_int, [C.c_void_p, C.c_int, C.c_int, C.c_int, C.c_int, C.c_void_p, C.c_void_p, C.c_void_p, C.c_void_p]),
diff --git a/rapiddoc_amd/build.py b/rapiddoc_amd/build.py
--- a/rapiddoc_amd/build.py
+++ b/rapiddoc_amd/build.py
@@ -10,7 +10,7 @@
 PKG = Path(__file__).resolve().parent
 CSRC = PKG / "csrc"
 OUT = PKG / "librapiddoc_mi355.so"
-SOURCES = ["kernels_conv.hip", "kernels_conv_h3.hip", "kernels_conv_direct_h3.hip", "kernels_conv3x3_h1.hip", "kernels_conv9x9_h1.hip", "kernels_stem34.hip", "kernels_rtdetr.hip", "kernels_conv_stream_h3.hip", "kernels_gemm_h3_dma.hip", "kernels_gemm_h1.hip", "kernels_misc.hip", "kernels_dw_lds.hip", "kernels_stem_fused.hip", "kernels_image.hip", "kernels_resize_aa.hip", "kernels_dbpost.hip", "kernels_checkbox.hip", "kernels_region.hip", "kernels_stage.hip", "kernels_attention_h3.hip", "kernels_seqconv.hip", "kernels_det_local.hip", "kernels_lcv3.hip", "kernels_lcv3_det.hip", "kernels_mv1e.hip", "kernels_mbv3.hip", "kernels_mbv3s.hip", "kernels_vit_attn.hip", "kernels_lcv3_block.hip", "kernels_ctc.hip", "kernels_mixer.hip", "kernels_mixer_h3.hip", "kernels_mixer_ws.hip", "kernels_mixer_res.hip", "formula_decoder.hip", "table_decoder.hip", "engine.cpp", "builder.cpp", "builder_mobile.cpp", "models.cpp", "api.cpp", "api_debug.cpp", "db_postprocess.cpp", "layout_postprocess.cpp", "polygon_ops.cpp", "checkbox_host.cpp", "rec_chunks.cpp", "host_stages.cpp", "stage_pack.cpp"]
+SOURCES = ["kernels_conv.hip", "kernels_conv_h3.hip", "kernels_conv_direct_h3.hip", "kernels_conv3x3_h1.hip", "kernels_conv9x9_h1.hip", "kernels_stem34.hip", "kernels_rtdetr.hip", "kernels_conv_stream_h3.hip", "kernels_gemm_h3_dma.hip", "kernels_gemm_h1.hip", "kernels_misc.hip", "kernels_dw_lds.hip", "kernels_stem_fused.hip", "kernels_image.hip", "kernels_resize_aa.hip", "kernels_dbpost.hip", "kernels_checkbox.hip", "kernels_region.hip", "kernels_stage.hip", "kernels_attention_h3.hip", "kernels_seqconv.hip", "kernels_det_local.hip", "kernels_lcv3.hip", "kernels_lcv3_det.hip", "kernels_mv1e.hip", "kernels_mbv3.hip", "kernels_mbv3s.hip", "kernels_vit_attn.hip", "kernels_lcv3_block.hip", "kernels_ctc.hip", "kernels_mixer.hip", "kernels_mixer_h3.hip", "kernels_mixer_ws.hip", "kernels_mixer_res.hip", "formula_decoder.hip", "table_decoder.hip", "engine.cpp", "builder.cpp", "builder_mobile.cpp", "models.cpp", "api.cpp", "api_debug.cpp", "db_postprocess.cpp", "layout_postprocess.cpp", "polygon_ops.cpp", "checkbox_host.cpp", "rec_chunks.cpp", "rec_plan.cpp", "host_stages.cpp", "stage_pack.cpp"]
 FLAGS = ["--offload-arch=gfx950", "-O3", "-std=c++17", "-fPIC", "-Wall", "-Wno-unused-function", "-x", "hip"]
 FILE_FLAGS = {"kernels_mixer_ws.hip": ["-fno-slp-vectorize", "-DRD_GELU_SCALAR"], "kernels_gemm_h1.hip": ["-fno-slp-vectorize"],
               "kernels_stem_fused.hip": ["-fno-slp-vectorize"]}
diff --git a/rapiddoc_amd/csrc/rec_plan.cpp b/rapiddoc_amd/csrc/rec_plan.cpp
--- /dev/null
+++ b/rapiddoc_amd/csrc/rec_plan.cpp
@@ -0,0 +1,418 @@
+#include <algorithm>
+#include <cmath>
+#include <cstdint>
+#include <cstring>
+#include <numeric>
+#include <utility>
+#include <vector>
+
+#include "../../include/rapiddoc_mi355.h"
+
+#pragma clang fp contract(off)
+
+namespace {
+
+constexpr int kImgH = 48, kImgW = 320;
+constexpr int kClsH = 48, kClsW = 192;
+constexpr int kNMin = 16, kNMax = 160, kNStep = 2;
+constexpr int kLaunchMultiple = 32;
+constexpr int kRefBatch = 6;
+constexpr int64_t kEqMaxColumns = 64 * 1088, kEqNMax = 160;
+constexpr int64_t kLineBucket = 32, kTBucket = 8, kTokenBucket = 256;
+constexpr int64_t kAlign = 64, kLinetabLines = 256;
+
+inline int64_t floordiv(int64_t a, int64_t b) {
+    int64_t q = a / b;
+    if ((a % b != 0) && ((a < 0) != (b < 0))) --q;
+    return q;
+}
+inline int64_t ceil_to(int64_t a, int64_t m) { return floordiv(a + m - 1, m) * m; }
+inline int32_t to_i32(double v) { return (v > -2147483649.0 && v < 2147483648.0) ? (int32_t)v : INT32_MIN; }
+inline int32_t low32(int64_t v) { return (int32_t)(uint32_t)(uint64_t)v; }
+
+inline float norm32(const float* a, const float* b) {
+    const float d0 = a[0] - b[0], d1 = a[1] - b[1];
+    const float s0 = d0 * d0, s1 = d1 * d1;
+    const float s = s0 + s1;
+    return std::sqrt(s);
+}
+inline float np_max(float a, float b) { return (a != a) ? a : (b != b) ? b : (a > b ? a : b); }
+
+struct LineDesc {
+    int32_t page, out_w, crop_w, crop_h, rot90, scratch_off;
+    double m[9];
+};
+static_assert(sizeof(LineDesc) == 96, "LINE_DTYPE is 96 bytes");
+
+}
+
+extern "C" int rd_rec_crop_systems(const double* quads, int n, double* cw_out, double* ch_out, uint8_t* ok_out, double* A_out, double* b_out,
+                                   int64_t* keep_out, int32_t* rot_out, double* ratio_out, int32_t* n_keep_out) {
+    if (!n_keep_out || n < 0) return 1;
+    *n_keep_out = 0;
+    if (n == 0) return 0;
+    if (!quads || !cw_out || !ch_out || !ok_out || !A_out || !b_out || !keep_out || !rot_out || !ratio_out) return 1;
+    int32_t n_keep = 0;
+    for (int i = 0; i < n; ++i) {
+        float q32[8];
+        double q[8];
+        for (int c = 0; c < 8; ++c) {
+            q32[c] = (float)quads[(size_t)i * 8 + c];
+            q[c] = (double)q32[c];
+        }
+        double cw = std::floor((double)np_max(norm32(q32 + 0, q32 + 2), norm32(q32 + 4, q32 + 6)));
+        double ch = std::floor((double)np_max(norm32(q32 + 0, q32 + 6), norm32(q32 + 2, q32 + 4)));
+        bool ok = cw >= 1.0 && ch >= 1.0 && std::isfinite(cw) && std::isfinite(ch);
+        if (!ok) cw = ch = 1.0;
+        static const int tri[4][3] = {{0, 1, 2}, {1, 2, 3}, {2, 3, 0}, {3, 0, 1}};
+        const double bound = 1e-6 * cw * ch;
+        for (const auto& t : tri) {
+            const double* pi = q + 2 * t[0];
+            const double* pj = q + 2 * t[1];
+            const double* pk = q + 2 * t[2];
+            const double l = (pj[0] - pi[0]) * (pk[1] - pi[1]);
+            const double r = (pj[1] - pi[1]) * (pk[0] - pi[0]);
+            const double cross = l - r;
+            ok = ok && std::isfinite(cross) && std::fabs(cross) > bound;
+        }
+        cw_out[i] = cw;
+        ch_out[i] = ch;
+        ok_out[i] = ok ? 1 : 0;
+        double* A = A_out + (size_t)i * 64;
+        double* b = b_out + (size_t)i * 8;
+        std::fill(A, A + 64, 0.0);
+        const double sx[4] = {0.0, cw, cw, 0.0}, sy[4] = {0.0, 0.0, ch, ch};
+        for (int p = 0; p < 4; ++p) {
+            const double x = sx[p], y = sy[p], u = q[2 * p], v = q[2 * p + 1];
+            b[2 * p] = u;
+            b[2 * p + 1] = v;
+            if (!ok) continue;
+            double* r0 = A + (2 * p) * 8;
+            double* r1 = r0 + 8;
+            r0[0] = x; r0[1] = y; r0[2] = 1.0; r0[6] = (-u) * x; r0[7] = (-u) * y;
+            r1[3] = x; r1[4] = y; r1[5] = 1.0; r1[6] = (-v) * x; r1[7] = (-v) * y;
+        }
+        if (!ok) {
+            for (int d = 0; d < 8; ++d) A[d * 8 + d] = 1.0;
+            continue;
+        }
+        const int32_t rot = (ch / cw >= 2.0) ? 1 : 0;
+        keep_out[n_keep] = i;
+        rot_out[n_keep] = rot;
+        ratio_out[n_keep] = rot ? ch / cw : cw / ch;
+        ++n_keep;
+    }
+    *n_keep_out = n_keep;
+    return 0;
+}
+
+extern "C" int rd_rec_plan(const double* cw, const double* ch, const int32_t* src_of, const int32_t* page_of, const double* mats, int n_all,
+                           const int64_t* keep, const int32_t* rot, const double* ratios, const int64_t* order, const int64_t* given_w,
+                           const double* given_ratio, int n, const int32_t* cfg, int64_t* line_i64_out, double* line_f64_out,
+                           int64_t* launch_out, int64_t* jobs_out, int64_t* group_out, int64_t* meta_out, uint8_t* block, int64_t block_bytes) {
+    if (!cfg || !meta_out || n < 1 || n_all < n) return 1;
+    if (!cw || !ch || !src_of || !page_of || !mats || !keep || !rot || !ratios || !order || !line_i64_out || !line_f64_out || !launch_out ||
+        !jobs_out || !group_out || block_bytes < 0 || (block_bytes > 0 && !block))
+        return 1;
+    const int mode = cfg[0];
+    const bool lines_in_launch = cfg[1] != 0, strict = cfg[2] != 0, use_cls = cfg[3] != 0, two_stage = cfg[4] != 0;
+    const int n_sources = cfg[5], rec_batch_num = cfg[6], width_multiple = cfg[7], n_cu = cfg[8], S = cfg[9];
+    if (mode < RD_REC_PLAN_LINES || mode > RD_REC_PLAN_FIXED || n_sources < 1 || rec_batch_num < 1 || width_multiple < 1 || S < 1) return 1;
+    if (mode == RD_REC_PLAN_LINES_GIVEN && (!given_w || !given_ratio)) return 1;
+    const bool lines_mode = mode == RD_REC_PLAN_LINES || mode == RD_REC_PLAN_LINES_GIVEN;
+    const size_t N = (size_t)n;
+    for (size_t i = 0; i < N; ++i) {
+        if (order[i] < 0 || order[i] >= n || keep[i] < 0 || keep[i] >= n_all) return 1;
+        if (n_sources > 1 && (src_of[keep[i]] < 0 || src_of[keep[i]] >= n_sources)) return 1;
+    }
+    int64_t* order_all = line_i64_out;
+    int64_t* line_ids = line_i64_out + N;
+    int64_t* line_w = line_i64_out + 2 * N;
+    int64_t* seq_line = line_i64_out + 3 * N;
+    int64_t* first_tok = line_i64_out + 4 * N;
+    double* crop_w = line_f64_out;
+    double* crop_h = line_f64_out + N;
+    double* eff_w = line_f64_out + 2 * N;
+    double* eff_h = line_f64_out + 3 * N;
+    double* line_ratio = line_f64_out + 4 * N;
+    const size_t L = N + 1;
+    int64_t* sizes = launch_out;
+    int64_t* widths = launch_out + L;
+    int64_t* starts = launch_out + 2 * L;
+    int64_t* batch_base = launch_out + 3 * L;
+    int64_t* tok_lo = launch_out + 4 * L;
+    int64_t* group_base = group_out;
+    int64_t* group_T = group_out + L;
+    int64_t* group_n = group_out + 2 * L;
+    int64_t* group_off = group_out + 3 * L;
+
+    for (size_t i = 0; i < N; ++i) {
+        const int64_t k = keep[i];
+        crop_w[i] = cw[k];
+        crop_h[i] = ch[k];
+        eff_w[i] = rot[i] == 1 ? ch[k] : cw[k];
+        eff_h[i] = rot[i] == 1 ? cw[k] : ch[k];
+        line_ratio[i] = 0.0;
+    }
+
+    std::vector<std::pair<int64_t, int64_t>> launches;
+    const double floor_ratio = (double)kImgW / (double)kImgH;
+    if (lines_mode) {
+        std::vector<int32_t> sz(N), lw(N);
+        int32_t n_out = 0;
+        if (mode == RD_REC_PLAN_LINES) {
+            if (rd_rec_plan_lines(ratios, order, n, kRefBatch, kImgH, kImgW, kLaunchMultiple, kNMin, kNMax, kNStep, n_cu, line_w, line_ratio,
+                                  sz.data(), lw.data(), n, &n_out) != 0)
+                return 4;
+        } else {
+            std::vector<int32_t> w32(N);
+            for (size_t i = 0; i < N; ++i) {
+                line_w[i] = given_w[order[i]];
+                line_ratio[i] = given_ratio[order[i]];
+                w32[i] = low32(floordiv(line_w[i] + kLaunchMultiple - 1, kLaunchMultiple) * kLaunchMultiple);
+            }
+            if (rd_rec_plan_chunks(w32.data(), n, kNMin, kNMax, kNStep, n_cu, sz.data(), n, &n_out) != 0) return 5;
+            int64_t i = 0;
+            for (int c = 0; c < n_out; ++c) {
+                i += sz[c];
+                lw[c] = w32[i - 1];
+            }
+        }
+        std::copy(order, order + N, order_all);
+        if (lines_in_launch) {
+            for (int c = 0; c < n_out; ++c) launches.push_back({sz[c], lw[c]});
+        } else {
+            for (int64_t i = 0; i < n;) {
+                const int64_t w = line_w[i];
+                int64_t j = i;
+                while (j < n && line_w[j] == w) ++j;
+                const int64_t cap = std::max<int64_t>(6, std::min(kEqNMax, floordiv(kEqMaxColumns, std::max<int64_t>(w, 1))));
+                for (int64_t a = i; a < j; a += cap) launches.push_back({std::min(a + cap, j) - a, w});
+                i = j;
+            }
+        }
+    } else if (mode == RD_REC_PLAN_ADAPTIVE) {
+        std::vector<int64_t> wp(N);
+        std::vector<int32_t> w32(N), sz(N);
+        for (size_t i = 0; i < N; ++i) {
+            const double r = ratios[order[i]];
+            const double wd = (double)kImgH * ((r != r) ? r : (floor_ratio > r ? floor_ratio : r));
+            if (!(wd > -2147483648.0 && wd < 2147483647.0 - width_multiple)) return 1;
+            wp[i] = (int64_t)wd;
+            if (width_multiple > 1) wp[i] = floordiv(wp[i] + width_multiple - 1, width_multiple) * width_multiple;
+            w32[i] = (int32_t)wp[i];
+        }
+        int32_t n_out = 0;
+        if (rd_rec_plan_chunks(w32.data(), n, kNMin, kNMax, kNStep, n_cu, sz.data(), n, &n_out) != 0) return 5;
+        int64_t i = 0;
+        for (int c = 0; c < n_out; ++c) {
+            i += sz[c];
+            launches.push_back({sz[c], wp[i - 1]});
+        }
+        std::copy(order, order + N, order_all);
+    } else {
+        std::vector<std::pair<int64_t, int64_t>> chunks;
+        for (int64_t beg = 0; beg < n; beg += rec_batch_num) {
+            const int64_t end = std::min<int64_t>(n, beg + rec_batch_num);
+            double r = ratios[order[beg]];
+            for (int64_t i = beg + 1; i < end; ++i)
+                if (ratios[order[i]] > r) r = ratios[order[i]];
+            if (!(r > floor_ratio)) r = floor_ratio;
+            const double wd = (double)kImgH * r;
+            if (!(wd > -2147483648.0 && wd < 2147483647.0 - width_multiple)) return 1;
+            int64_t w = (int64_t)wd;
+            if (width_multiple > 1) w = floordiv(w + width_multiple - 1, width_multiple) * width_multiple;
+            chunks.push_back({beg, w});
+        }
+        if (!strict) {
+            for (const auto& c : chunks) launches.push_back({std::min<int64_t>(n, c.first + rec_batch_num) - c.first, c.second});
+            std::copy(order, order + N, order_all);
+        } else {
+            std::vector<char> done(chunks.size(), 0);
+            int64_t pos = 0;
+            for (size_t a = 0; a < chunks.size(); ++a) {
+                if (done[a]) continue;
+                const int64_t first = pos;
+                for (size_t c = a; c < chunks.size(); ++c) {
+                    if (done[c] || chunks[c].second != chunks[a].second) continue;
+                    done[c] = 1;
+                    const int64_t end = std::min<int64_t>(n, chunks[c].first + rec_batch_num);
+                    for (int64_t i = chunks[c].first; i < end; ++i) order_all[pos++] = order[i];
+                }
+                launches.push_back({pos - first, chunks[a].second});
+            }
+        }
+    }
+    const int64_t nb = (int64_t)launches.size();
+    if (nb < 1 || nb > n) return 1;
+    starts[0] = 0;
+    for (int64_t b = 0; b < nb; ++b) {
+        sizes[b] = launches[b].first;
+        widths[b] = launches[b].second;
+        starts[b + 1] = starts[b] + sizes[b];
+        if (!lines_mode)
+            for (int64_t j = starts[b]; j < starts[b + 1]; ++j) line_w[j] = widths[b];
+    }
+    if (starts[nb] != n) return 1;
+
+    int64_t ng = 0;
+    std::vector<std::vector<int64_t>> dummy;
+    if (two_stage) {
+        for (size_t j = 0; j < N; ++j) {
+            const int64_t w2 = floordiv(line_w[j] - 1, 2) + 1;
+            seq_line[j] = floordiv(floordiv(w2 - 1, 2) + 1, 2);
+        }
+        ng = (nb + S - 1) / S;
+        dummy.resize((size_t)ng);
+        group_base[0] = 0;
+        for (int64_t g = 0; g < ng; ++g) {
+            const int64_t lo = starts[g * S], hi = starts[std::min<int64_t>(nb, (g + 1) * S)];
+            int64_t tok = 0, longest = seq_line[lo];
+            for (int64_t j = lo; j < hi; ++j) {
+                tok += seq_line[j];
+                longest = std::max(longest, seq_line[j]);
+            }
+            const int64_t nl = hi - lo;
+            const int64_t T = -floordiv(-longest, kTBucket) * kTBucket;
+            if (T < 1) return 1;
+            int64_t d = (nl / kLineBucket + 1) * kLineBucket - nl;
+            int64_t pad;
+            for (;;) {
+                pad = -floordiv(-(tok + d), kTokenBucket) * kTokenBucket - tok;
+                if (pad <= d * T) break;
+                d += kLineBucket;
+            }
+            const int64_t base = pad / d, extra = pad % d;
+            dummy[g].assign((size_t)d, base);
+            for (int64_t e = 0; e < extra; ++e) dummy[g][e] += 1;
+            group_T[g] = T;
+            group_n[g] = nl + d;
+            group_base[g + 1] = group_base[g] + tok + pad;
+            int64_t t = group_base[g];
+            for (int64_t j = lo; j < hi; ++j) {
+                first_tok[j] = t;
+                t += seq_line[j];
+            }
+        }
+        for (int64_t b = 0; b < nb; ++b) tok_lo[b] = first_tok[starts[b]];
+    }
+
+    const bool has_linetab = two_stage && lines_mode && lines_in_launch, has_warp = n_sources > 1;
+    int64_t off = 0;
+    const int64_t off_linetab = has_linetab ? off : -1;
+    if (has_linetab) off += 16 * ceil_to(n, kLinetabLines);
+    for (int64_t g = 0; g < ng; ++g) {
+        group_off[g] = off;
+        off = ceil_to(off + 4 * (2 * group_n[g] + (group_base[g + 1] - group_base[g])), kAlign);
+    }
+    const int64_t desc_bytes = ceil_to((int64_t)sizeof(LineDesc) * n, kAlign);
+    const int64_t off_descs = off;
+    off += desc_bytes;
+    const int64_t off_warp = has_warp ? off : -1;
+    if (has_warp) off += desc_bytes;
+    const int64_t off_cls = use_cls ? off : -1;
+    if (use_cls) off += desc_bytes;
+    meta_out[0] = nb;
+    meta_out[1] = ng;
+    meta_out[2] = 0;
+    meta_out[3] = off;
+    meta_out[4] = off_descs;
+    meta_out[5] = off_warp;
+    meta_out[6] = off_cls;
+    meta_out[7] = off_linetab;
+    if (off > block_bytes) return 2;
+
+    LineDesc* descs = reinterpret_cast<LineDesc*>(block + off_descs);
+    std::vector<int64_t> crop_px(N);
+    batch_base[0] = 0;
+    for (int64_t b = 0; b < nb; ++b) {
+        int64_t o = 0;
+        for (int64_t j = starts[b]; j < starts[b + 1]; ++j) {
+            const int64_t i = order_all[j];
+            if (i < 0 || i >= n) return 1;
+            line_ids[j] = keep[i];
+            LineDesc& d = descs[j];
+            d.page = page_of[keep[i]];
+            const double rw = std::ceil((double)kImgH * (eff_w[i] / eff_h[i]));
+            const double lwd = (double)line_w[j];
+            d.out_w = to_i32(lwd < rw ? lwd : rw);
+            d.crop_w = to_i32(crop_w[i]);
+            d.crop_h = to_i32(crop_h[i]);
+            d.rot90 = rot[i];
+            std::memcpy(d.m, mats + (size_t)keep[i] * 9, sizeof d.m);
+            crop_px[j] = (int64_t)d.crop_w * d.crop_h;
+            d.scratch_off = low32(o);
+            o += floordiv(crop_px[j] * 3 + 15, 16) * 16;
+        }
+        if (o >= ((int64_t)1 << 31)) return 3;
+        batch_base[b + 1] = batch_base[b] + o;
+    }
+
+    int64_t n_jobs = 0;
+    auto add_job = [&](int64_t b, int64_t src, int64_t first, int64_t cnt, int64_t max_px) {
+        int64_t* j = jobs_out + 5 * n_jobs++;
+        j[0] = b; j[1] = src; j[2] = first; j[3] = cnt; j[4] = max_px;
+    };
+    if (!has_warp) {
+        for (int64_t b = 0; b < nb; ++b)
+            add_job(b, 0, starts[b], sizes[b], *std::max_element(crop_px.begin() + starts[b], crop_px.begin() + starts[b + 1]));
+    } else {
+        LineDesc* warp = reinterpret_cast<LineDesc*>(block + off_warp);
+        std::vector<int64_t> idx;
+        for (int64_t b = 0; b < nb; ++b) {
+            const int64_t lo = starts[b], hi = starts[b + 1];
+            idx.resize((size_t)(hi - lo));
+            std::iota(idx.begin(), idx.end(), lo);
+            auto src = [&](int64_t j) { return src_of[keep[order_all[j]]]; };
+            std::stable_sort(idx.begin(), idx.end(), [&](int64_t a, int64_t c) { return src(a) < src(c); });
+            for (int64_t a = lo; a < hi;) {
+                int64_t e = a, max_px = crop_px[idx[a - lo]];
+                while (e < hi && src(idx[e - lo]) == src(idx[a - lo])) {
+                    warp[e] = descs[idx[e - lo]];
+                    max_px = std::max(max_px, crop_px[idx[e - lo]]);
+                    ++e;
+                }
+                add_job(b, src(idx[a - lo]), a, e - a, max_px);
+                a = e;
+            }
+        }
+        std::memset(reinterpret_cast<uint8_t*>(warp + N), 0, (size_t)(desc_bytes - (int64_t)sizeof(LineDesc) * n));
+    }
+    meta_out[2] = n_jobs;
+    std::memset(reinterpret_cast<uint8_t*>(descs + N), 0, (size_t)(desc_bytes - (int64_t)sizeof(LineDesc) * n));
+
+    if (use_cls) {
+        LineDesc* cls = reinterpret_cast<LineDesc*>(block + off_cls);
+        std::memcpy(cls, descs, (size_t)desc_bytes);
+        for (size_t j = 0; j < N; ++j) {
+            const int64_t i = order_all[j];
+            const double rw = std::ceil((double)kClsH * (eff_w[i] / eff_h[i]));
+            cls[j].out_w = to_i32((double)kClsW < rw ? (double)kClsW : rw);
+        }
+    }
+    if (has_linetab) {
+        int32_t* tab = reinterpret_cast<int32_t*>(block + off_linetab);
+        for (size_t j = 0; j < N; ++j) {
+            const int64_t w = line_w[j], w2 = floordiv(w - 1, 2) + 1, w4 = floordiv(w2 - 1, 2) + 1;
+            tab[4 * j] = low32(w); tab[4 * j + 1] = low32(w2); tab[4 * j + 2] = low32(w4); tab[4 * j + 3] = low32(first_tok[j]);
+        }
+        std::memset(tab + 4 * N, 0, (size_t)(16 * (ceil_to(n, kLinetabLines) - n)));
+    }
+    for (int64_t g = 0; g < ng; ++g) {
+        int32_t* seg = reinterpret_cast<int32_t*>(block + group_off[g]);
+        int32_t* tokinfo = seg + 2 * group_n[g];
+        const int64_t lo = starts[g * S], nl = starts[std::min<int64_t>(nb, (g + 1) * S)] - lo;
+        int64_t t = 0;
+        for (int64_t l = 0; l < group_n[g]; ++l) {
+            const int64_t len = l < nl ? seq_line[lo + l] : dummy[g][(size_t)(l - nl)];
+            seg[2 * l] = low32(t);
+            seg[2 * l + 1] = low32(len);
+            for (int64_t p = 0; p < len; ++p) tokinfo[t + p] = low32(p | (int64_t)((uint64_t)len << 16));
+            t += len;
+        }
+        const int64_t used = group_off[g] + 4 * (2 * group_n[g] + t);
+        const int64_t end = g + 1 < ng ? group_off[g + 1] : off_descs;
+        std::memset(block + used, 0, (size_t)(end - used));
+    }
+    return 0;
+}
diff --git a/rapiddoc_amd/pipeline.py b/rapiddoc_amd/pipeline.py
--- a/rapiddoc_amd/pipeline.py
+++ b/rapiddoc_amd/pipeline.py
@@ -12,7 +12,7 @@
 
 from . import _lib, ocr_host
 from .engine import RdEngine, preproc_resize_norm, preproc_resize_norm_batch
-from .rec_plan import (CLS_IMG_H, CLS_IMG_W, LINE_DTYPE, RecPlan, plan_rec,
+from .rec_plan import (CLS_IMG_H, CLS_IMG_W, LINE_DTYPE, RecPlan, StageBuffer, plan_rec,
                        quad_to_crop_matrix, quads_to_crop_matrices)
 
 LAYOUT_SIZE = 800
@@ -48,6 +48,17 @@
     lines: List[Tuple[np.ndarray, str, float]] = field(default_factory=list)
     layout_feats: Optional[List[torch.Tensor]] = None
     cls: Optional[List[Tuple[bool, int, float]]] = None
+
+
+class PinnedStageBuffer(StageBuffer):
+
+    def __init__(self):
+        super().__init__()
+        self.tensor = torch.empty(0, dtype=torch.uint8)
+
+    def alloc(self, nbytes: int) -> np.ndarray:
+        self.tensor = torch.empty(nbytes, dtype=torch.uint8, pin_memory=True)
+        return self.tensor.numpy()
 
 
 @dataclass(slots=True)
@@ -112,6 +123,9 @@
         self.prefetch_gate = float(os.environ.get("RD_PREFETCH_GATE", "1.0"))
         self.layout = RdEngine("pphgnetv2_b4", device, guard="deferred", reuse_outputs=True).load_weights(states["pphgnetv2_b4"]) if "pphgnetv2_b4" in states else None
         self._bufs: Dict[tuple, torch.Tensor] = {}
+        self._rec_stage = PinnedStageBuffer()
+        self._rec_stage_copied: Optional[torch.cuda.Event] = None
+        self._rec_stage_bytes = 0
         ncls = self.rec.num_classes
         self.characters = list(characters) if characters is not None else ["blank"] + [chr(0x4E00 + i) for i in range(ncls - 2)] + [" "]
         assert len(self.characters) == ncls, (len(self.characters), ncls)
@@ -235,10 +249,12 @@
         sync = None
         if self.rec_width_sync is not None and strict and self.rec_two_stage and self._sync_this_call:
             sync = lambda keys, ratios: self._synced_widths(self.rec_width_sync, keys, ratios)
+        if self._rec_stage_copied is not None:
+            self._rec_stage_copied.synchronize()
         plan = plan_rec([(imgs.shape[0], quads) for imgs, quads in sources], image_keys, strict=strict, two_stage=self.rec_two_stage,
                         lines_in_launch=self.rec_lines_in_launch, chunking=self.rec_chunking, rec_batch_num=self.rec_batch_num,
                         rec_width_multiple=self.rec_width_multiple, n_cu=self.n_cu, n_streams=len(self.rec_engines), use_cls=self.use_cls,
-                        host_native=self.host_native, want_words=want_words, width_sync=sync)
+                        host_native=self.host_native, want_words=want_words, width_sync=sync, stage=self._rec_stage)
         scatter = lambda per_line: self._scatter_texts(per_line, plan.src_of, plan.page_of, plan.n_img, plan.perm)
         cls_of: List[tuple] = [(False, 0, 0.0)] * plan.n_all
         if plan.n == 0:
@@ -275,19 +291,26 @@
         return scatter(texts)
 
     def _enqueue_rec(self, plan: RecPlan, sources, want_words: bool) -> List[_RecLaunch]:
-        dev, S, lib = sources[0][0].device, len(self.rec_engines), self._lib
+        S, lib = len(self.rec_engines), self._lib
         keep_inputs = self.keep_rec_inputs
-        upload = lambda descs: torch.from_numpy(descs.view(np.uint8)).to(dev, non_blocking=True)
-        descs_dev = upload(plan.descs)
+        main = torch.cuda.current_stream()
+        stage = plan.stage
+        host = self._rec_stage.tensor[: stage.nbytes]
+        assert host.data_ptr() == stage.block.ctypes.data
+        stage_dev = self._buf("rec_stage", stage.nbytes, torch.uint8)
+        stage_dev.copy_(host, non_blocking=True)
+        self._rec_stage_copied = torch.cuda.Event()
+        self._rec_stage_copied.record(main)
+        self._rec_stage_bytes = stage.nbytes
+        descs_dev = stage_dev[stage.descs_off:]
         cls = None
         if self.use_cls:
-            cls = (upload(plan.descs_cls), self._buf("cls_prob", 2 * plan.n).view(plan.n, 2), self._buf("cls_flip", plan.n, torch.int32),
+            cls = (stage_dev[stage.cls_off:], self._buf("cls_prob", 2 * plan.n).view(plan.n, 2), self._buf("cls_flip", plan.n, torch.int32),
                    torch.empty((plan.n, 2), dtype=torch.float32, pin_memory=True), torch.empty((plan.n,), dtype=torch.int32, pin_memory=True))
-        descs_warp_dev = upload(plan.descs_warp) if plan.descs_warp is not None else descs_dev
+        descs_warp_dev = stage_dev[stage.warp_off:] if plan.descs_warp is not None else descs_dev
         if keep_inputs:
             self.last_rec_descs = (plan.descs.copy(), np.asarray(plan.batch_base, dtype=np.int64), np.asarray(plan.starts, dtype=np.int64))
             self.last_cls_inputs = []
-        main = torch.cuda.current_stream()
         ready = torch.cuda.Event()
         ready.record(main)
         tokens = linetab = tables = None
@@ -296,13 +319,9 @@
             tokens = self._buf("rec_tokens", int(base[-1]) * self.rec.rec_token_dim).view(int(base[-1]), self.rec.rec_token_dim)
             for gi, lens in enumerate(plan.group_lens):
                 tokens[int(base[gi]) + int(lens.sum()): int(base[gi + 1])].zero_()
-            tables = [self.rec_tail.rec_tail_tables(lp, dev, out=self._buf(("tail_tab", gi), 2 * len(lp) + int(lp.sum()), torch.int32))
-                      for gi, (lp, _t) in enumerate(plan.group_pad)]
+            tables = [stage_dev[off: off + 4 * words].view(torch.int32) for off, words in zip(stage.group_off, stage.group_words)]
             if plan.linetab is not None:
-                tab_h = torch.from_numpy(plan.linetab).pin_memory()
-                linetab = self._buf("rec_linetab", 4 * plan.n, torch.int32).view(plan.n, 4)
-                linetab.copy_(tab_h, non_blocking=True)
-                self._keep_linetab = tab_h
+                linetab = stage_dev[stage.linetab_off: stage.linetab_off + 16 * plan.n].view(torch.int32).view(plan.n, 4)
             ready.record(main)
             self.tail_stream.wait_event(ready)
         launches: List[_RecLaunch] = []
diff --git a/rapiddoc_amd/rec_plan.py b/rapiddoc_amd/rec_plan.py
--- a/rapiddoc_amd/rec_plan.py
+++ b/rapiddoc_amd/rec_plan.py
@@ -1,12 +1,14 @@
 from __future__ import annotations
 
+import ctypes as C
+import os
 from dataclasses import dataclass
 from typing import Callable, List, Optional, Sequence, Tuple
 
 import numpy as np
 
-from . import ocr_host
-from .engine import pad_tail_lengths, rec_line_table
+from . import _lib, ocr_host
+from .engine import pad_tail_lengths, ragged_tables, rec_line_table
 
 CLS_IMG_H, CLS_IMG_W = 48, 192
 
@@ -98,6 +100,7 @@
     first_tok: Optional[np.ndarray] = None
     tok_lo: Optional[List[int]] = None
     linetab: Optional[np.ndarray] = None
+    stage: Optional["RecStage"] = None
 
     @property
     def n(self) -> int:
@@ -106,6 +109,99 @@
     @property
     def scratch_bytes(self) -> int:
         return int(self.batch_base[-1])
+
+
+STAGE_ALIGN, STAGE_LINETAB_LINES = 64, 256
+
+
+class StageBuffer:
+
+    def __init__(self):
+        self.array = np.empty(0, np.uint8)
+
+    def alloc(self, nbytes: int) -> np.ndarray:
+        return np.empty(nbytes, np.uint8)
+
+    def get(self, nbytes: int) -> np.ndarray:
+        if len(self.array) < nbytes:
+            self.array = self.alloc(int(nbytes * 1.25) + 4096)
+        return self.array
+
+
+@dataclass
+class RecStage:
+    block: np.ndarray
+    n: int
+    descs_off: int
+    warp_off: int
+    cls_off: int
+    linetab_off: int
+    group_off: List[int]
+    group_words: List[int]
+
+    @property
+    def nbytes(self) -> int:
+        return len(self.block)
+
+    def _descs(self, off: int) -> Optional[np.ndarray]:
+        return None if off < 0 else self.block[off: off + LINE_DTYPE.itemsize * self.n].view(LINE_DTYPE)
+
+    @property
+    def descs(self) -> np.ndarray:
+        return self._descs(self.descs_off)
+
+    @property
+    def descs_warp(self) -> Optional[np.ndarray]:
+        return self._descs(self.warp_off)
+
+    @property
+    def descs_cls(self) -> Optional[np.ndarray]:
+        return self._descs(self.cls_off)
+
+    @property
+    def linetab(self) -> Optional[np.ndarray]:
+        return None if self.linetab_off < 0 else self.block[self.linetab_off: self.linetab_off + 16 * self.n].view(np.int32).reshape(self.n, 4)
+
+    def tables(self, gi: int) -> np.ndarray:
+        return self.block[self.group_off[gi]: self.group_off[gi] + 4 * self.group_words[gi]].view(np.int32)
+
+
+def stage_layout(n: int, has_linetab: bool, group_words: Sequence[int], has_warp: bool, has_cls: bool):
+    up = lambda x, m: -(-x // m) * m
+    off = 0
+    linetab_off = -1
+    if has_linetab:
+        linetab_off, off = off, off + 16 * up(n, STAGE_LINETAB_LINES)
+    group_off = []
+    for words in group_words:
+        group_off.append(off)
+        off = up(off + 4 * int(words), STAGE_ALIGN)
+    desc_bytes = up(LINE_DTYPE.itemsize * n, STAGE_ALIGN)
+    descs_off, off = off, off + desc_bytes
+    warp_off = cls_off = -1
+    if has_warp:
+        warp_off, off = off, off + desc_bytes
+    if has_cls:
+        cls_off, off = off, off + desc_bytes
+    return descs_off, warp_off, cls_off, linetab_off, group_off, off
+
+
+def stage_plan(plan: RecPlan, buffer: Optional[StageBuffer] = None) -> None:
+    n = plan.n
+    words = [2 * len(lp) + int(lp.sum()) for lp, _t in plan.group_pad] if plan.two_stage else []
+    descs_off, warp_off, cls_off, linetab_off, group_off, total = stage_layout(
+        n, plan.linetab is not None, words, plan.descs_warp is not None, plan.descs_cls is not None)
+    block = (buffer or StageBuffer()).get(total)[:total]
+    block[:] = 0
+    st = RecStage(block, n, descs_off, warp_off, cls_off, linetab_off, group_off, words)
+    for name in ("descs", "descs_warp", "descs_cls", "linetab"):
+        if getattr(plan, name) is not None:
+            getattr(st, name)[...] = getattr(plan, name)
+            setattr(plan, name, getattr(st, name))
+    for gi, (lp, _t) in enumerate(plan.group_pad or []):
+        seg, tokinfo = ragged_tables(lp)
+        st.tables(gi)[...] = np.concatenate([seg.reshape(-1), tokinfo])
+    plan.stage = st
 
 
 def _no_lines(sync, **pooling) -> RecPlan:
@@ -117,7 +213,7 @@
 def plan_rec(sources: Sequence[Tuple[int, Sequence[np.ndarray]]], image_keys: Optional[Sequence[Sequence[int]]] = None, *,
              strict: bool, two_stage: bool, lines_in_launch: bool, chunking: str, rec_batch_num: int, rec_width_multiple: int,
              n_cu: int, n_streams: int, use_cls: bool = False, host_native: bool = True, want_words: bool = False,
-             width_sync: Optional[Callable] = None) -> RecPlan:
+             width_sync: Optional[Callable] = None, stage: Optional[StageBuffer] = None) -> RecPlan:
     z32 = np.zeros(0, np.int32)
     n_img = [int(k) for k, _q in sources]
     src_of, page_of, quad_list = [], [], []
@@ -137,6 +233,11 @@
         key = np.array([image_keys[si][pi] for si, pi in zip(src_of.tolist(), page_of.tolist())], dtype=np.int64)
         perm = np.argsort(key, kind="stable")
         quads, src_of, page_of, key = quads[perm], src_of[perm], page_of[perm], key[perm]
+    if host_native and os.environ.get("RD_REC_PLANNER", "dp") == "dp":
+        return _plan_rec_native(quads, src_of, page_of, perm, key if image_keys is not None else None, n_img, len(sources), strict=strict,
+                                two_stage=two_stage, lines_in_launch=lines_in_launch, chunking=chunking, rec_batch_num=rec_batch_num,
+                                rec_width_multiple=rec_width_multiple, n_cu=n_cu, n_streams=n_streams, use_cls=use_cls,
+                                want_words=want_words, width_sync=width_sync, stage=stage)
     mats, cws_a, chs_a, ok = quads_to_crop_matrices(quads)
     keep = np.nonzero(ok)[0]
     n = len(keep)
@@ -211,6 +312,7 @@
         plan.descs_cls["out_w"] = np.minimum(CLS_IMG_W, np.ceil(CLS_IMG_H * (eff_w / eff_h)[order_all])).astype(np.int32)
     if two_stage:
         _plan_tokens(plan, n_streams)
+    stage_plan(plan, stage)
     return plan
 
 
@@ -230,3 +332,98 @@
     plan.tok_lo = [int(first_tok[int(starts[bi])]) for bi in range(nb)]
     if plan.lines_in_launch:
         plan.linetab = rec_line_table(plan.line_w, first_tok)
+
+
+_MODE_LINES, _MODE_LINES_GIVEN, _MODE_ADAPTIVE, _MODE_FIXED = 0, 1, 2, 3
+
+
+def crop_systems_native(quads: np.ndarray):
+    quads = np.ascontiguousarray(quads, dtype=np.float64).reshape(-1, 4, 2)
+    n = len(quads)
+    cw, ch, ok = np.empty(n), np.empty(n), np.empty(n, np.uint8)
+    A, b = np.empty((n, 8, 8)), np.empty((n, 8))
+    keep, rot, ratio = np.empty(n, np.int64), np.empty(n, np.int32), np.empty(n)
+    k = C.c_int32(0)
+    rc = _lib.load().rd_rec_crop_systems(quads.ctypes.data, n, cw.ctypes.data, ch.ctypes.data, ok.ctypes.data, A.ctypes.data, b.ctypes.data,
+                                         keep.ctypes.data, rot.ctypes.data, ratio.ctypes.data, C.byref(k))
+    if rc != 0:
+        raise RuntimeError("rd_rec_crop_systems failed")
+    return cw, ch, ok, A, b, keep[: k.value], rot[: k.value], ratio[: k.value]
+
+
+def _plan_rec_native(quads, src_of, page_of, perm, key, n_img, n_sources, *, strict, two_stage, lines_in_launch, chunking, rec_batch_num,
+                     rec_width_multiple, n_cu, n_streams, use_cls, want_words, width_sync, stage) -> RecPlan:
+    lib = _lib.load()
+    n_all = len(quads)
+    cw, ch, _ok, A, b, keep, rot, ratio = crop_systems_native(quads)
+    n = len(keep)
+    pooling = dict(n_img=n_img, src_of=src_of, page_of=page_of, perm=perm, keep=keep, n_all=n_all)
+    if n == 0:
+        return _no_lines(width_sync, **pooling)
+    mats = np.empty((n_all, 9))
+    mats[:, :8] = np.linalg.solve(A, b[..., None])[..., 0]
+    mats[:, 8] = 1.0
+    lines_mode = strict and two_stage
+    if want_words and not lines_mode:
+        raise RuntimeError("word boxes need the strict two-stage recogniser (rec_mode='strict', RD_REC_TWO_STAGE unset)")
+    gw = gr = None
+    if lines_mode:
+        mode = _MODE_LINES
+        if width_sync is not None:
+            line_keys = key[keep] if key is not None else page_of[keep].astype(np.int64)
+            given = width_sync(line_keys, ratio.copy())
+            gw, gr = np.ascontiguousarray(given[0], dtype=np.int64), np.ascontiguousarray(given[1], dtype=np.float64)
+            assert len(gw) == len(gr) == n
+            mode = _MODE_LINES_GIVEN
+            order = np.lexsort((ratio, gw))
+        else:
+            order = np.argsort(ratio)
+    elif not strict and chunking == "adaptive":
+        mode, order = _MODE_ADAPTIVE, np.argsort(ratio, kind="stable")
+    else:
+        mode, order = _MODE_FIXED, (np.argsort(ratio) if strict else np.argsort(ratio, kind="stable"))
+    order = np.ascontiguousarray(order, dtype=np.int64)
+    src_of, page_of = np.ascontiguousarray(src_of, dtype=np.int32), np.ascontiguousarray(page_of, dtype=np.int32)
+    cfg = np.array([mode, lines_in_launch, strict, use_cls, two_stage, n_sources, rec_batch_num, rec_width_multiple, n_cu, n_streams], np.int32)
+    li, lf = np.empty((5, n), np.int64), np.empty((5, n))
+    launch, jobs, group, meta = np.empty((5, n + 1), np.int64), np.empty((n, 5), np.int64), np.empty((4, n + 1), np.int64), np.zeros(8, np.int64)
+    buffer = stage or StageBuffer()
+    need = 3 * LINE_DTYPE.itemsize * n + 16 * (n + STAGE_LINETAB_LINES) + 8 * n
+    while True:
+        block = buffer.get(need)
+        rc = lib.rd_rec_plan(cw.ctypes.data, ch.ctypes.data, src_of.ctypes.data, page_of.ctypes.data, mats.ctypes.data, n_all,
+                             keep.ctypes.data, rot.ctypes.data, ratio.ctypes.data, order.ctypes.data,
+                             None if gw is None else gw.ctypes.data, None if gr is None else gr.ctypes.data, n, cfg.ctypes.data,
+                             li.ctypes.data, lf.ctypes.data, launch.ctypes.data, jobs.ctypes.data, group.ctypes.data, meta.ctypes.data,
+                             block.ctypes.data, len(block))
+        if rc != 2 or int(meta[3]) <= len(block):
+            break
+        need = int(meta[3])
+    if rc == 3:
+        raise RuntimeError("a rec batch needs >= 2 GB of crop scratch: lower rec_batch_num")
+    if rc != 0:
+        raise RuntimeError({4: "rd_rec_plan_lines failed", 5: "rd_rec_plan_chunks failed"}.get(rc, "rd_rec_plan failed"))
+    nb, ng, n_jobs, total = (int(v) for v in meta[:4])
+    starts = launch[2, : nb + 1]
+    cuts = starts.tolist()
+    order_all = li[0]
+    words = [2 * lines + tok for lines, tok in zip(group[2, :ng].tolist(), np.diff(group[0, : ng + 1]).tolist())]
+    st = RecStage(block[:total], n, int(meta[4]), int(meta[5]), int(meta[6]), int(meta[7]), group[3, :ng].tolist(), words)
+    plan = RecPlan(**pooling, lines_mode=lines_mode, two_stage=two_stage, lines_in_launch=lines_mode and lines_in_launch,
+                   crop_w=lf[0], crop_h=lf[1], rot90=rot, eff_w=lf[2], eff_h=lf[3], ratios=ratio.tolist(),
+                   order_all=order_all, line_ids=li[1], line_w=li[2], line_ratio=lf[4] if lines_mode else None,
+                   batches=[(order_all[a:e], w) for a, e, w in zip(cuts[:-1], cuts[1:], launch[1, :nb].tolist())], starts=starts,
+                   descs=st.descs, descs_cls=st.descs_cls, descs_warp=st.descs_warp, batch_base=launch[3, : nb + 1], stage=st)
+    plan.warp_jobs = [[] for _ in range(nb)]
+    for bi, si, first, cnt, max_px in jobs[:n_jobs].tolist():
+        plan.warp_jobs[bi].append((si, first, cnt, max_px))
+    if two_stage:
+        S = n_streams
+        plan.seq_line, plan.first_tok, plan.tok_lo = li[3], li[4], launch[4, :nb].tolist()
+        plan.groups = [list(range(g, min(g + S, nb))) for g in range(0, nb, S)]
+        plan.group_lens = [plan.seq_line[cuts[grp[0]]: cuts[grp[-1] + 1]] for grp in plan.groups]
+        plan.group_pad = [(st.tables(gi)[1: 2 * lines: 2].astype(np.int64), T)
+                          for gi, (lines, T) in enumerate(zip(group[2, :ng].tolist(), group[1, :ng].tolist()))]
+        plan.group_base = group[0, : ng + 1]
+        plan.linetab = st.linetab
+    return plan
```

After: 379.0, median of 6. 1.01x the previous value.
